# SeanNaren/deepspeech.pytorch

Measured on AMD Instinct MI355X. Metric: audio-seconds/sec (train step), higher is better.
Workload: dtype bf16

## Files before the change

deepspeech/pytorch_amd/_lib.py:

```python
import ctypes as C
import os

HERE = os.path.dirname(os.path.abspath(__file__))
LIB_PATH = os.path.join(HERE, "libds2hip.so")

F32, BF16 = 0, 1
CELL_GRU, CELL_LSTM, CELL_RNN_TANH = 0, 1, 2

_vp, _i, _l, _f, _ll = C.c_void_p, C.c_int, C.c_long, C.c_float, C.c_longlong

SIGNATURES = {
    "ds2_version": (_i, []),
    "ds2_error_string": (C.c_char_p, [_i]),
    "ds2_gemm_nt": (_i, [_i, _vp, _vp, _vp, _vp, _i, _i, _i, _l, _l, _l, _i, _i, _l, _l, _l, _l, _i, _vp]),
    "ds2_gemm_nt_coresident": (_i, [_i, _vp, _vp, _vp, _vp, _i, _i, _i, _l, _l, _l, _i, _i, _l, _l, _l, _l, _i, _vp]),
    "ds2_gemm_nt_rows2": (_i, [_i, _vp, _vp, _i, _vp, _vp, _i, _i, _i, _l, _l, _l, _i, _i, _i, _vp]),
    "ds2_gemm8_nt": (_i, [_vp, _vp, _vp, _vp, _i, _i, _i, _l, _l, _l, _i, _vp]),
    "ds2_gemm8_tn_grouped": (_i, [_i, _vp, _vp, _vp, _vp, _vp, _vp, _vp, _vp, _vp, _vp, _vp, _i, _vp]),
    "ds2_gemm8_nt_rows": (_i, [_vp, _vp, _vp, _vp, _i, _i, _i, _l, _l, _l, _i, _vp, _i, _vp]),
    "ds2_gemm8_tn_grouped_rows": (_i, [_i, _vp, _vp, _vp, _vp, _vp, _vp, _vp, _vp, _vp, _vp, _vp, _i, _vp, _i, _vp]),
    "ds2_gemm8_wgrad_dx_rows": (_i, [_i, _vp, _vp, _vp, _vp, _vp, _vp, _vp, _vp, _vp, _vp, _vp, _i, _vp, _vp, _vp, _i, _i, _i, _l, _l, _l, _vp, _i, _vp]),
    "ds2_zero_pad_rows": (_i, [_i, _vp, _l, _i, _vp, _i, _i, _vp]),
    "ds2_gemm8_wgrad_dx": (_i, [_i, _vp, _vp, _vp, _vp, _vp, _vp, _vp, _vp, _vp, _vp, _vp, _i, _vp, _vp, _vp, _i, _i, _i, _l, _l, _l, _vp]),
    "ds2_norm_partials": (_i, [_l]),
    "ds2_bn_fwd": (_i, [_i, _i, _i, _vp, _vp, _l, _i, _l, _l, _i, _i, _i, _vp, _vp, _vp, _vp, _vp, _vp, _f, _f, _vp, _vp,
                        _vp, _vp, _vp, _vp]),
    "ds2_bn_bwd": (_i, [_i, _i, _vp, _vp, _vp, _l, _i, _l, _l, _l, _i, _i, _i, _vp, _vp, _vp, _vp, _vp, _vp, _vp, _vp, _vp]),
    "ds2_colsum": (_i, [_i, _vp, _l, _i, _l, _vp, _f, _vp, _vp]),
    "ds2_conv_rows": (_i, [_i, _vp, _vp]),
    "ds2_conv1_fwd": (_i, [_i, _vp, _vp, _vp, _vp, _vp, _i, _i, _i, _i, _vp]),
    "ds2_conv1_wgrad_ws_floats": (_l, [_i, _i, _i]),
    "ds2_conv1_wgrad": (_i, [_i, _vp, _vp, _vp, _i, _i, _i, _i, _vp, _vp]),
    "ds2_conv2_fwd_ws_bytes": (_l, [_i, _i, _i, _i]),
    "ds2_conv2_fwd": (_i, [_i, _vp, _vp, _vp, _vp, _vp, _i, _i, _i, _vp, _vp]),
    "ds2_conv2_dgrad": (_i, [_i, _vp, _vp, _vp, _vp, _i, _i, _i, _vp]),
    "ds2_conv2_wgrad_ws_floats": (_l, [_i, _i]),
    "ds2_conv2_wgrad": (_i, [_i, _vp, _vp, _vp, _i, _i, _i, _vp, _vp]),
    "ds2_rnn_gates": (_i, [_i]),
    "ds2_rnn_saved_planes": (_i, [_i]),
    "ds2_rnn_state_bytes": (_l, [_i, _i, _i]),
    "ds2_rnn_fwd": (_i, [_i, _i, _i, _i, _i, _i, _vp, _vp, _vp, _vp, _vp, _vp, _vp, _l, _vp, _vp, _vp, _vp, _vp]),
    "ds2_rnn_bwd": (_i, [_i, _i, _i, _i, _i, _i, _vp, _vp, _vp, _vp, _l, _vp, _vp, _vp, _vp, _vp, _vp, _vp, _vp, _vp]),
    "ds2_rnn_persist_plan": (_i, [_i, _i, _i, _i, _i, _i, C.c_uint, C.POINTER(_l)]),
    "ds2_rnn_persist_supported": (_i, [_i, _i, _i, _i, _i, C.c_uint]),
    "ds2_rnn_persist_shape_covered": (_i, [_i, _i, _i, _i, _i]),
    "ds2_rnn_persist_kind": (_i, [_i, _i, _i, _i, _i, C.c_uint]),
    "ds2_rnn_persist_ws_bytes": (_l, [_i, _i, _i, _i, _i, C.c_uint]),
    "ds2_rnn_persist_fwd": (_i, [_i, _i, _i, _i, _i, _i, _vp, _vp, _vp, _vp, _vp, _vp, _vp, _l, _vp, _vp, _vp, _vp, _vp, _vp, _vp]),
    "ds2_rnn_persist_bwd": (_i, [_i, _i, _i, _i, _i, _i, _vp, _vp, _vp, _vp, _l, _vp, _vp, _vp, _vp, _i, _vp, _vp, _vp, _vp]),
    "ds2_add2": (_i, [_i, _vp, _vp, _vp, _l, _vp]),
    "ds2_sum_slices": (_i, [_vp, _vp, _l, _i, _vp]),
    "ds2_transpose": (_i, [_i, _vp, _vp, _l, _i, _l, _l, _vp]),
    "ds2_split3_bf16": (_i, [_vp, _l, _l, _i, _i, _i, _vp, _l, _vp]),
    "ds2_cast_transpose_bf16": (_i, [_vp, _l, _i, _i, _i, _i, _i, _vp, _l, _vp, _l, _vp]),
    "ds2_small_weight_layouts": (_i, [_i, _vp, _vp, _vp, _i, _i, _vp, _vp, _vp, _vp, _vp, _vp, _vp]),
    "ds2_scale_by": (_i, [_vp, _vp, _l, _vp]),
    "ds2_copy_words": (_i, [_vp, _vp, _l, _vp]),
    "ds2_lookahead_fwd": (_i, [_i, _vp, _vp, _vp, _vp, _i, _i, _i, _i, _vp]),
    "ds2_lookahead_ws_floats": (_l, [_i, _i, _i, _i]),
    "ds2_lookahead_bwd": (_i, [_i, _vp, _vp, _vp, _vp, _vp, _vp, _i, _i, _i, _i, _vp, _vp]),
    "ds2_rnn_bias_grads": (_i, [_i, _i, _i, _i, _vp, _vp, _vp, _vp]),
    "ds2_fc_supported": (_i, [_i, _i]),
    "ds2_fc_fwd": (_i, [_vp, _l, _vp, _l, _vp, _l, _l, _i, _i, _vp]),
    "ds2_fc_bwd_partials": (_l, [_l, _l]),
    "ds2_fc_bwd": (_i, [_vp, _l, _vp, _l, _vp, _l, _vp, _l, _vp, _vp, _l, _i, _i, _l, _vp]),
    "ds2_softmax_rows": (_i, [_vp, _vp, _l, _i, _l, _l, _vp]),
    "ds2_opt_max_tensors": (_i, []),
    "ds2_clip_ws_floats": (_l, [_i, _vp]),
    "ds2_clip_coef": (_i, [_i, _vp, _vp, _f, _vp, _vp, _vp]),
    "ds2_opt_multi": (_i, [_i, _i, _vp, _vp, _vp, _vp, _vp, _vp, _i, _vp, _vp]),
    "ds2_opt_matrix": (_i, [_i, _vp, _vp, _vp, _vp, _i, _i, _i, _i, _i, _vp, _l, _vp, _l, _vp, _i, _vp, _vp]),
    "ds2_opt_matrices": (_i, [_i, _i] + [_vp] * 13 + [_vp, _i, _vp, _vp]),
    "ds2_spect_frames": (_i, [_i]),
    "ds2_spect_ws_bytes": (_l, [_i, _i]),
    "ds2_spectrogram": (_i, [_vp, _l, _vp, _i, _i, _vp, _i, _i, _vp, _vp, _vp]),
    "ds2_spectrogram_aug": (_i, [_vp, _l, _vp, _i, _i, _vp, _i, _i, _vp, _vp, _vp, _i, _vp, _i, _vp, _i, _vp, _vp]),
    "ds2_spec_augment_coef": (_i, [_vp, _i, _i, _i, _vp, _vp, _i, _vp, _vp]),
    "ds2_spec_augment": (_i, [_vp, _vp, _i, _i, _i, _vp, _vp, _vp, _i, _vp, _i, _vp]),
    "ds2_wsola_segments": (_i, [_i, _f]),
    "ds2_wsola_out_len": (_l, [_i, _f]),
    "ds2_wsola": (_i, [_vp, _l, _vp, _vp, _i, _vp, _l, _vp, _vp, _i, _vp]),
    "ds2_wave_ws_bytes": (_l, [_i]),
    "ds2_wave_energy": (_i, [_vp, _l, _vp, _i, _vp, _vp, _vp, _l, _vp, _vp, _vp, _vp]),
    "ds2_wave_mix": (_i, [_vp, _l, _vp, _i, _vp, _vp, _vp, _l, _vp, _vp, _vp, _vp, _l, _vp]),
    "ds2_greedy_decode":(_i, [_vp, _l, _l, _i, _i, _i, _vp, _i, _vp, _vp, _vp, _vp]),
    "ds2_beam_ws_bytes": (_l, [_i, _i, _i]),
    "ds2_beam_decode": (_i, [_vp, _l, _l, _i, _i, _i, _vp, _i, _i, _i, _f, _vp, _vp, _vp, _vp, _vp, _vp]),
    "ds2_beam_decode_lm": (_i, [_vp, _l, _l, _i, _i, _i, _vp, _i, _i, _i, _f, _i, _vp, _l, _vp, _l, _i, _i, _f, _f, _i,
                                _vp, _vp, _vp, _vp, _vp, _vp, _vp]),
    "ds2_beam_grid_ws_bytes": (_l, [_i, _i, _i, _i]),
    "ds2_beam_decode_lm_grid": (_i, [_vp, _l, _l, _i, _i, _i, _vp, _i, _i, _i, _f, _i, _vp, _l, _vp, _l, _i, _i, _i, _i, _vp, _vp,
                                     _vp, _vp, _vp, _vp, _vp, _vp, _vp]),
    "ds2_greedy_stream_feed": (_i, [_vp, _l, _l, _i, _i, _i, _vp, _i, _vp, _vp, _vp, _vp, _vp]),
    "ds2_beam_stream_bytes": (_l, [_i, _i, _i, _i]),
    "ds2_beam_stream_ws_bytes": (_l, [_i, _i]),
    "ds2_beam_stream_state_stride": (_l, [_i, _i]),
    "ds2_beam_stream_reset": (_i, [_vp, _i, _i, _i, _i, _vp, _vp]),
    "ds2_beam_stream_feed": (_i, [_vp, _l, _l, _i, _i, _i, _vp, _i, _i, _i, _f, _vp, _i, _vp, _vp, _l, _i, _vp, _vp, _vp, _vp]),
    "ds2_beam_stream_feed_lm": (_i, [_vp, _l, _l, _i, _i, _i, _vp, _i, _i, _i, _f, _i, _vp, _l, _vp, _l, _i, _i, _f, _f, _i,
                                     _vp, _i, _vp, _vp, _l, _i, _vp, _vp, _vp, _vp, _vp]),
    "ds2_stream_plan": (_i, [_l, _i, _i, _i, _vp]),
    "ds2_stream_state_bytes": (_l, [_i, _i, _i, _i, _i]),
    "ds2_stream_conv1": (_i, [_i, _vp, _vp, _vp, _vp, _vp, _vp, _vp, _vp, _vp, _vp, _i, _i, _i, _i, _i, _vp]),
    "ds2_stream_conv2": (_i, [_i, _vp, _vp, _vp, _vp, _vp, _vp, _vp, _vp, _vp, _vp, _i, _i, _i, _i, _i, _i, _vp]),
    "ds2_stream_lookahead": (_i, [_i, _vp, _vp, _vp, _vp, _vp, _vp, _i, _i, _i, _i, _i, _i, _vp]),
    "ds2_stream_conv1_rows": (_i, [_i, _vp, _vp, _vp, _vp, _vp, _vp, _vp, _vp, _vp, _i, _i, _i, _i, _vp]),
    "ds2_stream_conv2_rows": (_i, [_i, _vp, _vp, _vp, _vp, _vp, _vp, _vp, _vp, _vp, _i, _i, _i, _i, _i, _i, _vp]),
    "ds2_stream_lookahead_rows": (_i, [_i, _vp, _vp, _vp, _vp, _vp, _vp, _i, _i, _i, _i, _i, _i, _vp]),
    "ds2_error_counts": (_i, [_vp, _l, _vp, _i, _vp, _vp, _i, _i, _vp, _vp, _vp, _vp, _vp]),
    "ds2_ctc_ws_floats": (_l, [_i, _i, _i, _i]),
    "ds2_ctc_loss_grad": (_i, [_vp, _l, _vp, _vp, _vp, _vp, _i, _i, _i, _i, _i, _f, _vp, _vp, _vp, _l, _vp, _i, _vp]),
    "ds2_ctc_align_ws_bytes": (_l, [_i, _i, _i]),
    "ds2_ctc_align": (_i, [_vp, _l, _l, _i, _i, _i, _i, _vp, _vp, _vp, _vp, _i, _i, _vp, _vp, _vp, _vp, _vp, _vp, _vp]),
}



class PersistOpts(C.Structure):
    _fields_ = [("variant", C.c_uint), ("spin_limit", C.c_uint), ("startup_ms", C.c_uint)]


_lib = None


class Ds2HipError(RuntimeError):
    pass


def load():
    global _lib
    if _lib is not None:
        return _lib
    if not os.path.exists(LIB_PATH):
        raise Ds2HipError(
            "libds2hip.so not found at %s -- build it with `python -m deepspeech.pytorch_amd.build` "
            "(hipcc --offload-arch=gfx950).  There is no fallback path." % LIB_PATH)
    lib = C.CDLL(LIB_PATH)
    for name, (res, args) in SIGNATURES.items():
        fn = getattr(lib, name)
        fn.restype = res
        fn.argtypes = args
    _lib = lib
    return lib


def error_string(code):
    return load().ds2_error_string(int(code)).decode()


def call(name, *args):
    rc = getattr(load(), name)(*args)
    if rc != 0:
        raise Ds2HipError("%s failed with code %d: %s" % (name, rc, error_string(rc)))


def query(name, *args):
    return getattr(load(), name)(*args)
```

deepspeech/pytorch_amd/csrc/ds2_conv.hip:

```cpp
#include "ds2_common.h"

namespace {

constexpr int F0 = 161, F1 = 81, F2 = 41, CH = 32;
constexpr int K1F = 41, K1T = 11, K2F = 21, K2T = 11;

constexpr int C1_FB = 4, C1_TB = 64;
constexpr int C1_PR = (C1_FB - 1) * 2 + K1F;
constexpr int C1_PC = (C1_TB - 1) * 2 + K1T;
constexpr int C1_PCP = C1_PC + 1;

__device__ __forceinline__ void conv1_load_patch(float* patch, const float* __restrict__ xn, int T, int f_base, int t_base,
                                                 int tid, int nthreads, int f0) {
  for (int i = tid; i < C1_PR * C1_PC; i += nthreads) {
    const int pr = i / C1_PC, pc = i - pr * C1_PC;
    const int fi = f_base + pr, ti = t_base + pc;
    const bool ok = fi >= 0 && fi < f0 && ti >= 0 && ti < T;
    const float v = xn[(long)min(max(fi, 0), f0 - 1) * T + min(max(ti, 0), T - 1)];
    patch[pr * C1_PCP + pc] = ok ? v : 0.f;
  }
}

template <typename T>
__global__ void __launch_bounds__(256) k_conv1_fwd(const float* __restrict__ x, const float* __restrict__ w1k,
// ... 652 lines not shown
    cur.j = q0 - cur.n * NJ;
  }
  cur = next_live(cur);
  int b = 0;
  if (cur.n < N) {
    const CwdNext first = plan(cur, 0);
    cwd_dma_dy<KSN, 0>(first); cwd_dma_dy<KSN, 1>(first); cwd_dma_dy<KSN, 2>(first);
    if constexpr (KSN > 3) cwd_dma_dy<KSN, 3>(first);
    if constexpr (KSN > 4) cwd_dma_dy<KSN, 4>(first);
    if constexpr (KSN > 5) cwd_dma_dy<KSN, 5>(first);
    if constexpr (KSN > 6) cwd_dma_dy<KSN, 6>(first);
    if constexpr (KSN > 7) cwd_dma_dy<KSN, 7>(first);
    cwd_dma_x<KSN, 0>(first); cwd_dma_x<KSN, 1>(first); cwd_dma_x<KSN, 2>(first);
  }
  while (cur.n < N) {
    Cursor nc = cur;
    advance(nc);
    nc = next_live(nc);
    const CwdNext nx = plan(nc, b ^ 1);
    CWD_WAIT_VM0();
    __builtin_amdgcn_sched_barrier(0);
    __builtin_amdgcn_s_barrier();
    __builtin_amdgcn_sched_barrier(0);
    const uint32_t aA = la + b * BUF, aB = lb + b * BUF;
#define CWD_FIRST(IDX) CWD_READ(fa[0], fb[0], 0, IDX);
    CWD_FIRST(0) CWD_FIRST(1) CWD_FIRST(2) CWD_FIRST(3) CWD_FIRST(4) CWD_FIRST(5) CWD_FIRST(6)
    CWD_FIRST(7) CWD_FIRST(8) CWD_FIRST(9) CWD_FIRST(10) CWD_FIRST(11) CWD_FIRST(12) CWD_FIRST(13)
#undef CWD_FIRST
    cwd_kstep<KSN, 0>(acc, fa, fb, aA, aB, nx);
    cwd_kstep<KSN, 1>(acc, fa, fb, aA, aB, nx);
    cwd_kstep<KSN, 2>(acc, fa, fb, aA, aB, nx);
    if constexpr (KSN > 3) cwd_kstep<KSN, 3>(acc, fa, fb, aA, aB, nx);
    if constexpr (KSN > 4) cwd_kstep<KSN, 4>(acc, fa, fb, aA, aB, nx);
    if constexpr (KSN > 5) cwd_kstep<KSN, 5>(acc, fa, fb, aA, aB, nx);
    if constexpr (KSN > 6) cwd_kstep<KSN, 6>(acc, fa, fb, aA, aB, nx);
    if constexpr (KSN > 7) cwd_kstep<KSN, 7>(acc, fa, fb, aA, aB, nx);
    cur = nc;
    b ^= 1;
  }
#pragma unroll
  for (int r = 0; r < R; ++r)
#pragma unroll
    for (int i = 0; i < 3; ++i) {
      const int kt = wave + 4 * i;
      if (kt < K2T && kf0 + 2 * r < K2F) {
        float* out = partial + (((long)split * K2F + (kf0 + 2 * r)) * K2T + kt) * (CH * CH);
#pragma unroll
        for (int e = 0; e < 16; ++e) out[mma32_row(e, lane) * 32 + li] = acc[r][i][e];
      }
    }
}

struct RTapArgs {
  const bf16_t* X;
  const bf16_t* W;
  const float* bias;
  const int* lens;
  const float* Pin;
  float* Pout;
  bf16_t* Y;
  int N, Tp, Fin, Fout;
  int KF, WSF, WQ;
  int ISF, IQ, PF;
  int U, OSF, OQ;
};
constexpr int RT_FB = 4, RT_TB = 32, RT_PC = RT_TB + K2T - 1;
constexpr int RT_KFM = 11, RT_PR = RT_FB - 1 + RT_KFM;
constexpr int RT_PCD = 48, RT_ROWB = RT_PCD * CH * 2;
constexpr int RT_PATCH = RT_PR * RT_ROWB;
constexpr int RT_RED = 4 * RT_FB * 4096;
constexpr int RT_SMEM = 2 * RT_PATCH + RT_RED;
#define RT_RD128(dst, addr, off) asm volatile("ds_read_b128 %0, %1 offset:%2" : "=v"(dst) : "v"(addr), "i"(off))

struct RtNext {
  __amdgpu_buffer_rsrc_t rx;
  unsigned char* patch;
  int n, ub, tb;
  int Fin, Tp, PF, ISF, IQ;
  int wave, lane;
};
template <int PR, int I>
__device__ __forceinline__ void rt_dma_piece(const RtNext& nx) {
  constexpr int k = I % 3;
  const int pr = nx.wave + 4 * (I / 3);
  if (pr < PR) {
    const int fi = (nx.ub * RT_FB + pr - nx.PF) * nx.ISF + nx.IQ;
    const bool row_ok = nx.n >= 0 && fi >= 0 && fi < nx.Fin;
    const int soff = __builtin_amdgcn_readfirstlane(row_ok ? (nx.n * nx.Fin + fi) * (nx.Tp * CH * 2) : 0);
    const int pc = 16 * k + (nx.lane >> 2), ti = nx.tb * RT_TB - 5 + pc;
    const int voff = (row_ok && pc < RT_PC && (unsigned)ti < (unsigned)nx.Tp) ? ti * (CH * 2) + (((nx.lane & 3) ^ (nx.lane >> 4)) << 4) : CW_OOB;
    __builtin_amdgcn_raw_ptr_buffer_load_lds(nx.rx, (cw_lds_ptr_t)(nx.patch + pr * RT_ROWB + k * 1024), 16, voff, soff, 0, 0);
  }
}
template <int PR, int I>
__device__ __forceinline__ void rt_dma_all(const RtNext& nx) {
  rt_dma_piece<PR, I>(nx);
  if constexpr (I + 1 < 12) rt_dma_all<PR, I + 1>(nx);
}
constexpr int RT_AH = 4;
template <int ST>
__device__ __forceinline__ void rt_prefetch(uint4 (&bq)[RT_AH + 1], const uint32_t (&aj)[6]) {
  RT_RD128(bq[ST], aj[ST % 6], (ST / 6) * RT_ROWB);
  if constexpr (ST + 1 < RT_AH) rt_prefetch<ST + 1>(bq, aj);
}
template <int KF, int ST>
__device__ __forceinline__ void rt_step(ds2_f32x16 (&acc)[RT_FB], const uint4 (&A)[KF][6], uint4 (&bq)[RT_AH + 1], const uint32_t (&aj)[6],
                                        const RtNext& nx) {
  constexpr int PR = RT_FB - 1 + KF, NS = PR * 6, rho = ST / 6, j = ST % 6;
  if constexpr (ST + RT_AH < NS) RT_RD128(bq[(ST + RT_AH) % (RT_AH + 1)], aj[(ST + RT_AH) % 6], ((ST + RT_AH) / 6) * RT_ROWB);
  constexpr int left = RT_AH < NS - 1 - ST ? RT_AH : NS - 1 - ST;
  if constexpr (left >= 4) asm volatile("s_waitcnt lgkmcnt(4)" ::: "memory");
  else if constexpr (left == 3) asm volatile("s_waitcnt lgkmcnt(3)" ::: "memory");
  else if constexpr (left == 2) asm volatile("s_waitcnt lgkmcnt(2)" ::: "memory");
  else if constexpr (left == 1) asm volatile("s_waitcnt lgkmcnt(1)" ::: "memory");
  else asm volatile("s_waitcnt lgkmcnt(0)" ::: "memory");
  __builtin_amdgcn_sched_barrier(0);
#pragma unroll
  for (int fl = 0; fl < RT_FB; ++fl) {
    const int m = rho - fl;
    if (m >= 0 && m < KF) Mma<bf16_t>::mma32(acc[fl], A[m][j], bq[ST % (RT_AH + 1)]);
  }
  if constexpr (ST % 6 == 3 && ST >= 9 && (ST - 9) / 6 < 12) rt_dma_piece<PR, (ST - 9) / 6>(nx);
  __builtin_amdgcn_sched_barrier(0);
  if constexpr (ST + 1 < NS) rt_step<KF, ST + 1>(acc, A, bq, aj, nx);
}

template <int KF>
__global__ void __launch_bounds__(256, 1) k_conv_rtap(RTapArgs a) {
  extern __shared__ __attribute__((aligned(16))) unsigned char rsm[];
  float* red = reinterpret_cast<float*>(rsm + 2 * RT_PATCH);
  const int tid = threadIdx.x, lane = tid & 63, wave = __builtin_amdgcn_readfirstlane(tid >> 6);
  const int li = lane & 31, lq = lane >> 5;
  const int i0 = wave < 2 ? 6 * wave : 12 + 5 * (wave - 2), icnt = wave < 2 ? 6 : 5;
  uint4 A[KF][6];
  const uint32_t lds0 = (uint32_t)(uintptr_t)(__attribute__((address_space(3))) unsigned char*)rsm;
  uint32_t boff[6];
#pragma unroll
  for (int j = 0; j < 6; ++j) {
    const int item = i0 + min(j, icnt - 1), kt = item >> 1, half = item & 1;
    const int p = li + kt;
    boff[j] = lds0 + p * (CH * 2) + (((half * 2 + lq) ^ ((p >> 2) & 3)) << 4);
#pragma unroll
    for (int m = 0; m < KF; ++m) {
      const uint4 wv = *reinterpret_cast<const uint4*>(a.W + (((long)(m * a.WSF + a.WQ) * K2T + kt) * CH + li) * CH + half * 16 + lq * 8);
      A[m][j] = j < icnt ? wv : make_uint4(0u, 0u, 0u, 0u);
    }
  }
#ifndef DS2_RTAP_VKEEP
#define DS2_RTAP_VKEEP 24
#endif
#pragma unroll
  for (int m = 0; m < KF; ++m)
#pragma unroll
    for (int j = 0; j < 6; ++j)
      if (m * 6 + j >= DS2_RTAP_VKEEP) {
        typedef __attribute__((ext_vector_type(4))) unsigned int u4v;
        u4v v = __builtin_bit_cast(u4v, A[m][j]);
        asm volatile("" : "+a"(v));
        A[m][j] = __builtin_bit_cast(uint4, v);
      }
  constexpr int PR = RT_FB - 1 + KF;
  constexpr int NPIECE = 12;
  const int nub = ds2_cdiv_dev(a.U, RT_FB), ntb = ds2_cdiv_dev(a.Tp, RT_TB);
  const int total = a.N * nub * ntb;
  RtNext nx;
  nx.rx = __builtin_amdgcn_make_buffer_rsrc((void*)a.X, 0, a.N * a.Fin * a.Tp * CH * 2, 0x00020000);
  nx.Fin = a.Fin; nx.Tp = a.Tp; nx.PF = a.PF; nx.ISF = a.ISF; nx.IQ = a.IQ;
  nx.wave = wave; nx.lane = lane;
  auto aim = [&](int tile, int buf) {
    const bool any = tile < total;
    const int tt = any ? tile : 0;
    nx.tb = tt % ntb;
    nx.ub = (tt / ntb) % nub;
    nx.n = any ? tt / (ntb * nub) : -1;
    nx.patch = rsm + buf * RT_PATCH;
  };

  int tile = blockIdx.x;
  if (tile < total) {
    aim(tile, 0);
    rt_dma_all<PR, 0>(nx);
  }
  __syncthreads();
  int buf = 0;
  for (; tile < total; tile += gridDim.x, buf ^= 1) {
    const int tb = tile % ntb, ub = (tile / ntb) % nub, n = tile / (ntb * nub);
    const int next = tile + gridDim.x;
    aim(next, buf ^ 1);
    float4 pin[4];
    {
      const int u = ub * RT_FB + wave, t = tb * RT_TB + li;
      const bool have = a.Pin != nullptr && u < a.U && t < a.Tp;
      const float* src = a.Pin + (((long)n * a.U + min(u, a.U - 1)) * a.Tp + min(t, a.Tp - 1)) * CH + 4 * lq;
#pragma unroll
      for (int g = 0; g < 4; ++g) pin[g] = have ? *reinterpret_cast<const float4*>(src + 8 * g) : make_float4(0.f, 0.f, 0.f, 0.f);
    }
    ds2_f32x16 acc[RT_FB];
#pragma unroll
    for (int fl = 0; fl < RT_FB; ++fl)
#pragma unroll
      for (int r = 0; r < 16; ++r) acc[fl][r] = 0.f;
    {
      uint4 bq[RT_AH + 1];
      uint32_t aj[6];
#pragma unroll
      for (int j = 0; j < 6; ++j) aj[j] = boff[j] + buf * RT_PATCH;
      __builtin_amdgcn_sched_barrier(0);
      rt_prefetch<0>(bq, aj);
      rt_step<KF, 0>(acc, A, bq, aj, nx);
    }
#pragma unroll
    for (int fl = 0; fl < RT_FB; ++fl)
#pragma unroll
      for (int g = 0; g < 4; ++g)
        *reinterpret_cast<float4*>(red + (((wave * RT_FB + fl) * 4 + g) * 64 + lane) * 4) =
            make_float4(acc[fl][4 * g], acc[fl][4 * g + 1], acc[fl][4 * g + 2], acc[fl][4 * g + 3]);
    asm volatile("s_waitcnt vmcnt(0)" ::: "memory");
    __syncthreads();
    {
      const int u = ub * RT_FB + wave, t = tb * RT_TB + li;
      float o[16];
#pragma unroll
      for (int g = 0; g < 4; ++g) {
        float4 s4 = *reinterpret_cast<const float4*>(red + (((0 * RT_FB + wave) * 4 + g) * 64 + lane) * 4);
#pragma unroll
        for (int w = 1; w < 4; ++w) {
          const float4 q4 = *reinterpret_cast<const float4*>(red + (((w * RT_FB + wave) * 4 + g) * 64 + lane) * 4);
          s4.x += q4.x; s4.y += q4.y; s4.z += q4.z; s4.w += q4.w;
        }
        o[4 * g] = s4.x; o[4 * g + 1] = s4.y; o[4 * g + 2] = s4.z; o[4 * g + 3] = s4.w;
      }
      if (u < a.U && t < a.Tp) {
        const long pidx = (((long)n * a.U + u) * a.Tp + t) * CH + 4 * lq;
        if (a.Pin) {
#pragma unroll
          for (int g = 0; g < 4; ++g) {
            o[4 * g] += pin[g].x; o[4 * g + 1] += pin[g].y; o[4 * g + 2] += pin[g].z; o[4 * g + 3] += pin[g].w;
          }
        }
        if (a.Pout) {
#pragma unroll
          for (int g = 0; g < 4; ++g)
            *reinterpret_cast<float4*>(a.Pout + pidx + 8 * g) = make_float4(o[4 * g], o[4 * g + 1], o[4 * g + 2], o[4 * g + 3]);
        } else {
          const bool live = a.lens ? (t < a.lens[n]) : true;
          bf16_t* dst = a.Y + (((long)n * a.Fout + u * a.OSF + a.OQ) * a.Tp + t) * CH + 4 * lq;
#pragma unroll
          for (int g = 0; g < 4; ++g) {
            float e[4];
#pragma unroll
            for (int c = 0; c < 4; ++c) e[c] = live ? o[4 * g + c] + (a.bias ? a.bias[8 * g + 4 * lq + c] : 0.f) : 0.f;
            *reinterpret_cast<uint2*>(dst + 8 * g) = make_uint2(cvt_pk_bf16(e[0], e[1]), cvt_pk_bf16(e[2], e[3]));
          }
        }
      }
    }
    asm volatile("s_waitcnt lgkmcnt(0)" ::: "memory");
    __builtin_amdgcn_sched_barrier(0);
    __builtin_amdgcn_s_barrier();
    __builtin_amdgcn_sched_barrier(0);
  }
}

template <int KF>
int conv_rtap_launch_kf(const RTapArgs& a, hipStream_t st) {
  static bool attr[DS2_MAX_DEVICES];
  if (ds2_first_use_on_device(attr)) (void)hipFuncSetAttribute((const void*)k_conv_rtap<KF>, hipFuncAttributeMaxDynamicSharedMemorySize, RT_SMEM);
  const long total = (long)a.N * ds2_cdiv(a.U, RT_FB) * ds2_cdiv(a.Tp, RT_TB);
  const int cus = ds2_cu_count();
  hipLaunchKernelGGL(k_conv_rtap<KF>, dim3((unsigned)(total < cus ? total : cus)), dim3(256), RT_SMEM, st, a);
  DS2_CHECK_LAUNCH();
  return 0;
}
int conv_rtap_launch(const RTapArgs& a, hipStream_t st) {
  if (a.KF == 11) return conv_rtap_launch_kf<11>(a, st);
  if (a.KF == 10) return conv_rtap_launch_kf<10>(a, st);
  return DS2_ERR_ARG;
}

template <typename T, int NT>
int conv_tap_launch_nt(const ConvTapArgs& a, hipStream_t st) {
  const int PR = (CT_UB - 1) * a.SF + a.KF, PC = CT_TB * NT + K2T - 1;
  const int shm = PR * PC * CT_POSB + 2 * CT_WST_BYTES;
  static int attr[DS2_MAX_DEVICES];
  int dev = 0;
  (void)hipGetDevice(&dev);
  dev = dev >= 0 && dev < DS2_MAX_DEVICES ? dev : 0;
  if (attr[dev] < shm) {
    (void)hipFuncSetAttribute((const void*)k_conv_tap<T, NT>, hipFuncAttributeMaxDynamicSharedMemorySize, shm);
    attr[dev] = shm;
  }
  dim3 grid(ds2_cdiv(a.Tp, CT_TB * NT), ds2_cdiv(a.U, CT_UB), a.N);
  hipLaunchKernelGGL((k_conv_tap<T, NT>), grid, dim3(256), shm, st, a);
  DS2_CHECK_LAUNCH();
  return 0;
}
template <typename T>
int conv_tap_launch(const ConvTapArgs& a, hipStream_t st) {
  const int PR = (CT_UB - 1) * a.SF + a.KF;
  if (PR * (2 * CT_TB + K2T - 1) * CT_POSB + 2 * CT_WST_BYTES <= 150 * 1024) return conv_tap_launch_nt<T, 2>(a, st);
  return conv_tap_launch_nt<T, 1>(a, st);
}

}

static bool conv_geometry(int f0, int& f1, int& f2) {
  f1 = (f0 + 2 * 20 - K1F) / 2 + 1;
  f2 = (f1 + 2 * 10 - K2F) / 2 + 1;
  return f0 >= 1 && f1 >= 1 && f2 >= 1;
}

extern "C" {

int ds2_conv_rows(int F0, int* F1_out, int* F2_out) {
  int f1, f2;
  DS2_REQUIRE(conv_geometry(F0, f1, f2), DS2_ERR_ARG);
  if (F1_out) *F1_out = f1;
  if (F2_out) *F2_out = f2;
  return 0;
}

int ds2_conv1_fwd(int dtype, const float* x, const float* w1k, const float* b1, const int* lens, void* y1, int N, int F0_, int T,
                  int Tp, ds2_stream_t st_) {
  hipStream_t st = (hipStream_t)st_;
  DS2_REQUIRE(dtype == DS2_F32 || dtype == DS2_BF16, DS2_ERR_DTYPE);
  int f1, f2;
  DS2_REQUIRE(N > 0 && T > 0 && Tp == (T + 2 * 5 - 10 - 1) / 2 + 1 && conv_geometry(F0_, f1, f2), DS2_ERR_ARG);
  dim3 grid(ds2_cdiv(Tp, C1_TB), ds2_cdiv(f1, C1_FB), N);
  if (dtype == DS2_F32) {
    hipLaunchKernelGGL(k_conv1_fwd<float>, grid, dim3(256), 0, st, x, w1k, b1, lens, (float*)y1, N, T, Tp, F0_, f1);
  } else if (F0_ != F0) {
    hipLaunchKernelGGL(k_conv1_fwd<bf16_t>, grid, dim3(256), 0, st, x, w1k, b1, lens, (bf16_t*)y1, N, T, Tp, F0_, f1);
  } else {
    const int ntb = ds2_cdiv(Tp, M1_TB);
    const long total = (long)N * ntb * 9;
    const int cus = ds2_cu_count();
    hipLaunchKernelGGL(k_conv1_fwd_mfma, dim3((unsigned)(total < cus ? total : cus)), dim3(256), 0, st, x, w1k, b1, lens, (bf16_t*)y1, N,
                       T, Tp, ntb);
  }
  DS2_CHECK_LAUNCH();
  return 0;
}

static int conv1_wgrad_blocks(int N, int f1, int Tp) {
  long total = (long)N * ds2_cdiv(f1, C1_FB) * ds2_cdiv(Tp, C1_TB);
  return (int)(total < C1W_MAXBLOCKS ? total : C1W_MAXBLOCKS);
}
static int conv1_wgrad_mfma_blocks(int N, int Tp) {
  const long total = (long)N * ds2_cdiv(Tp, M1_TB) * 9;
  const int cus = ds2_cu_count();
  return (int)(total < cus ? total : cus);
}
long ds2_conv1_wgrad_ws_floats(int N, int F0_, int Tp) {
  int f1, f2;
  if (!conv_geometry(F0_, f1, f2)) return 0;
  const long P = conv1_wgrad_blocks(N, f1, Tp);
  return P * (K1F * K1T * CH) + (long)ds2_norm_partials(P) * (K1F * K1T * CH);
}
int ds2_conv1_wgrad(int dtype, const float* x, const void* dy1, float* dw1k, int N, int F0_, int T, int Tp, float* ws,
                    ds2_stream_t st_) {
  hipStream_t st = (hipStream_t)st_;
  DS2_REQUIRE(dtype == DS2_F32 || dtype == DS2_BF16, DS2_ERR_DTYPE);
  int f1, f2;
  DS2_REQUIRE(conv_geometry(F0_, f1, f2), DS2_ERR_ARG);
  int P = conv1_wgrad_blocks(N, f1, Tp);
  const int ncf = ds2_cdiv(f1, C1_FB), nct = ds2_cdiv(Tp, C1_TB);
  if (dtype == DS2_F32) {
    hipLaunchKernelGGL(k_conv1_wgrad<float>, dim3(P), dim3(C1W_THREADS), 0, st, x, (const float*)dy1, ws, N, T, Tp, nct, ncf, F0_, f1);
  } else if (F0_ != F0) {
    hipLaunchKernelGGL(k_conv1_wgrad<bf16_t>, dim3(P), dim3(C1W_THREADS), 0, st, x, (const bf16_t*)dy1, ws, N, T, Tp, nct, ncf, F0_, f1);
  } else {
    static bool attr[DS2_MAX_DEVICES];
    if (ds2_first_use_on_device(attr))
      (void)hipFuncSetAttribute((const void*)k_conv1_wgrad_mfma, hipFuncAttributeMaxDynamicSharedMemorySize, M1W_SMEM);
    P = conv1_wgrad_mfma_blocks(N, Tp) < P ? conv1_wgrad_mfma_blocks(N, Tp) : P;
    hipLaunchKernelGGL(k_conv1_wgrad_mfma, dim3(P), dim3(256), M1W_SMEM, st, x, (const bf16_t*)dy1, ws, N, T, Tp, ds2_cdiv(Tp, M1_TB));
  }
  DS2_CHECK_LAUNCH();
  const int C = K1F * K1T * CH;
  return ds2_colsum(DS2_F32, ws, P, C, C, dw1k, 1.0f, ws + (long)P * C, st_);
}

long ds2_conv2_fwd_ws_bytes(int dtype, int N, int F0_, int Tp) { return (dtype == DS2_BF16 && F0_ == F0) ? (long)N * F2 * Tp * CH * 4 : 0; }
int ds2_conv2_fwd(int dtype, const void* a1, const void* w2t, const float* b2, const int* lens, void* y2, int N, int F0_, int Tp, void* ws,
                  ds2_stream_t st_) {
  hipStream_t st = (hipStream_t)st_;
  DS2_REQUIRE(dtype == DS2_F32 || dtype == DS2_BF16, DS2_ERR_DTYPE);
  int f1, f2;
  DS2_REQUIRE(N > 0 && Tp > 0 && conv_geometry(F0_, f1, f2), DS2_ERR_ARG);
  if (dtype == DS2_F32 || F0_ != F0 || (long)N * F1 * Tp * CH * 2 >= (long)CW_OOB) {
    ConvTapArgs a{a1, w2t, b2, lens, y2, N, Tp, f1, f2, K2F, 2, 10, f2, 1, 0};
    return dtype == DS2_F32 ? conv_tap_launch<float>(a, st) : conv_tap_launch<bf16_t>(a, st);
  }
  DS2_REQUIRE(ws != nullptr, DS2_ERR_ARG);
  RTapArgs e{(const bf16_t*)a1, (const bf16_t*)w2t, nullptr, nullptr, nullptr, (float*)ws, nullptr, N, Tp, F1, F2, 11, 2, 0, 2, 0, 5, F2, 1, 0};
  RTapArgs o{(const bf16_t*)a1, (const bf16_t*)w2t, b2, lens, (const float*)ws, nullptr, (bf16_t*)y2, N, Tp, F1, F2, 10, 2, 1, 2, 1, 5, F2, 1, 0};
  const int rc = conv_rtap_launch(e, st);
  return rc ? rc : conv_rtap_launch(o, st);
}

int ds2_conv2_dgrad(int dtype, const void* dy2, const void* w2d_even, const void* w2d_odd, void* da1, int N, int F0_, int Tp,
                    ds2_stream_t st_) {
  hipStream_t st = (hipStream_t)st_;
  DS2_REQUIRE(dtype == DS2_F32 || dtype == DS2_BF16, DS2_ERR_DTYPE);
  int f1, f2;
  DS2_REQUIRE(N > 0 && Tp > 0 && conv_geometry(F0_, f1, f2), DS2_ERR_ARG);
  if (dtype == DS2_BF16 && F0_ == F0 && (long)N * F1 * Tp * CH * 2 < (long)CW_OOB) {
    RTapArgs e{(const bf16_t*)dy2, (const bf16_t*)w2d_even, nullptr, nullptr, nullptr, nullptr, (bf16_t*)da1, N, Tp, F2, F1, 11, 1, 0, 1, 0, 5, 41, 2, 0};
    RTapArgs o{(const bf16_t*)dy2, (const bf16_t*)w2d_odd, nullptr, nullptr, nullptr, nullptr, (bf16_t*)da1, N, Tp, F2, F1, 10, 1, 0, 1, 0, 4, 40, 2, 1};
    const int rc = conv_rtap_launch(e, st);
    return rc ? rc : conv_rtap_launch(o, st);
  }
  ConvTapArgs e{dy2, w2d_even, nullptr, nullptr, da1, N, Tp, f2, f1, 11, 1, 5, (f1 + 1) / 2, 2, 0};
  ConvTapArgs o{dy2, w2d_odd, nullptr, nullptr, da1, N, Tp, f2, f1, 10, 1, 4, f1 / 2, 2, 1};
  if (dtype == DS2_F32) {
    const int rc = conv_tap_launch<float>(e, st);
    return (rc || f1 / 2 == 0) ? rc : conv_tap_launch<float>(o, st);
  }
  const int rc = conv_tap_launch<bf16_t>(e, st);
  return (rc || f1 / 2 == 0) ? rc : conv_tap_launch<bf16_t>(o, st);
}

long ds2_conv2_wgrad_ws_floats(int N, int Tp) {
  (void)N; (void)Tp;
  const long C = (long)K2F * K2T * CH * CH;
  static_assert(CWR_SPLITS >= CW_SPLITS, "sized for the larger split count of the two kernels");
  return (long)CWR_SPLITS * C + (long)ds2_norm_partials(CWR_SPLITS) * C;
}
int ds2_conv2_wgrad(int dtype, const void* dy2, const void* a1, float* dw2t, int N, int F0_, int Tp, float* ws, ds2_stream_t st_) {
  hipStream_t st = (hipStream_t)st_;
  DS2_REQUIRE(dtype == DS2_F32 || dtype == DS2_BF16, DS2_ERR_DTYPE);
  int f1, f2;
  DS2_REQUIRE(conv_geometry(F0_, f1, f2), DS2_ERR_ARG);
  dim3 grid(K2F, CW_SPLITS);
  const bool general = dtype == DS2_F32 || F0_ != F0 || (long)N * F1 * Tp * CH * 2 >= (long)CW_OOB;
  if (dtype == DS2_F32) {
    hipLaunchKernelGGL(k_conv2_wgrad<float>, grid, dim3(256), 0, st, (const float*)dy2, (const float*)a1, ws, N, Tp, f1, f2);
  } else if (general) {
    hipLaunchKernelGGL(k_conv2_wgrad<bf16_t>, grid, dim3(256), 0, st, (const bf16_t*)dy2, (const bf16_t*)a1, ws, N, Tp, f1, f2);
  } else {
    static bool attr[DS2_MAX_DEVICES];
    constexpr int smem = cwd_smem_bytes(CWD_KSN);
    if (ds2_first_use_on_device(attr))
      (void)hipFuncSetAttribute((const void*)k_conv2_wgrad_bf16d<CWD_KSN>, hipFuncAttributeMaxDynamicSharedMemorySize, smem);
    hipLaunchKernelGGL(k_conv2_wgrad_bf16d<CWD_KSN>, dim3(8 * CWD_UNITS_PER_XCD), dim3(256), smem, st, (const bf16_t*)dy2, (const bf16_t*)a1, ws, N,
                       Tp, CWR_SPLITS);
  }
  DS2_CHECK_LAUNCH();
  const int C = K2F * K2T * CH * CH;
  const int splits = general ? CW_SPLITS : CWR_SPLITS;
  return ds2_colsum(DS2_F32, ws, splits, C, C, dw2t, 1.0f, ws + (long)splits * C, st_);
}

}
```

deepspeech/pytorch_amd/csrc/ds2_norm.hip:

```cpp
#include "ds2_common.h"

namespace {

constexpr int NORM_RY = 8;
constexpr int NORM_CX = 32;

struct RowMap {
  int F, Tp;
  __device__ __forceinline__ void nt(long row, int& n, int& t) const {
    t = (int)(row % Tp);
    n = (int)(row / ((long)F * Tp));
  }
};

__device__ __forceinline__ float bn_affine(float x, float sc, float sh) { return __builtin_fmaf(x, sc, sh); }
__device__ __forceinline__ bool hardtanh_open(float y) { return y > 0.f && y < 20.f; }
__device__ __forceinline__ float bn_dx(float g, float xh, float sc, float k1, float k2) { return sc * __builtin_fmaf(-xh, k2, g - k1); }

struct RedMap {
  int cpb, rpx, chunk, rsub;
  bool ok;
  __device__ __forceinline__ RedMap(int chunks) {
    cpb = chunks < NORM_CX ? chunks : NORM_CX;
    rpx = NORM_CX / cpb;
    const int tx = threadIdx.x;
    rsub = tx / cpb;
    chunk = blockIdx.x * cpb + tx % cpb;
    ok = rsub < rpx && chunk < chunks;
  }
  __device__ __forceinline__ long first_row() const { return ((long)blockIdx.y * NORM_RY + threadIdx.y) * rpx + rsub; }
  __device__ __forceinline__ long row_step() const { return (long)gridDim.y * NORM_RY * rpx; }
};
template <int V>
__device__ __forceinline__ void red_block(float (*red)[NORM_CX * V + 1], const RedMap& m, const float (&v)[V], float (&out)[V]) {
  __syncthreads();
#pragma unroll
  for (int i = 0; i < V; ++i) red[threadIdx.y][threadIdx.x * V + i] = v[i];
  __syncthreads();
  if (threadIdx.y == 0 && m.rsub == 0) {
#pragma unroll
    for (int i = 0; i < V; ++i) {
      float a = 0.f;
      for (int k = 0; k < m.rpx; ++k)
#pragma unroll
        for (int y = 0; y < NORM_RY; ++y) a += red[y][(threadIdx.x + k * m.cpb) * V + i];
      out[i] = a;
    }
  }
}

template <typename T, bool SQ>
__global__ void __launch_bounds__(NORM_RY* NORM_CX) k_colstats(const T* __restrict__ X, long R, int C, long ld,
                                                                float* __restrict__ psum, float* __restrict__ psq) {
  constexpr int V = Vec16<T>::N;
  __shared__ float red[NORM_RY][NORM_CX * V + 1];
  const RedMap m(C / V);
  float s[V], q[V];
#pragma unroll
  for (int i = 0; i < V; ++i) s[i] = q[i] = 0.f;
  if (m.ok) {
    for (long r = m.first_row(); r < R; r += m.row_step()) {
      float v[V];
      Vec16<T>::load(X + r * ld + (long)m.chunk * V, v);
#pragma unroll
      for (int i = 0; i < V; ++i) {
        s[i] += v[i];
        if (SQ) q[i] += v[i] * v[i];
      }
    }
  }
  float o[V];
  red_block<V>(red, m, s, o);
  if (threadIdx.y == 0 && m.rsub == 0 && m.ok) {
#pragma unroll
    for (int i = 0; i < V; ++i) psum[(long)blockIdx.y * C + (long)m.chunk * V + i] = o[i];
  }
  if (SQ) {
    red_block<V>(red, m, q, o);
    if (threadIdx.y == 0 && m.rsub == 0 && m.ok) {
#pragma unroll
      for (int i = 0; i < V; ++i) psq[(long)blockIdx.y * C + (long)m.chunk * V + i] = o[i];
    }
  }
}

constexpr int FIN_COLS = 32, FIN_SLICES = 8;
template <int NA>
__device__ __forceinline__ void finalize_sums(const float* const (&arr)[NA], int P, int C, int c, int py, double (&tot)[NA]) {
  __shared__ double sh[NA][FIN_SLICES][FIN_COLS];
  double acc[NA];
#pragma unroll
  for (int a = 0; a < NA; ++a) acc[a] = 0.0;
  if (c < C) {
#pragma unroll 8
    for (int p = py; p < P; p += FIN_SLICES) {
#pragma unroll
      for (int a = 0; a < NA; ++a) acc[a] += (double)arr[a][(long)p * C + c];
    }
  }
#pragma unroll
  for (int a = 0; a < NA; ++a) sh[a][py][threadIdx.x & (FIN_COLS - 1)] = acc[a];
  __syncthreads();
#pragma unroll
  for (int a = 0; a < NA; ++a) {
    double t = 0.0;
    if (py == 0) {
#pragma unroll
      for (int q = 0; q < FIN_SLICES; ++q) t += sh[a][q][threadIdx.x & (FIN_COLS - 1)];
    }
    tot[a] = t;
  }
}

__global__ void __launch_bounds__(256) k_colsum_finalize(const float* __restrict__ psum, int P, int C, float* __restrict__ out,
                                                          float scale) {
  const int c = blockIdx.x * FIN_COLS + (threadIdx.x & (FIN_COLS - 1)), py = threadIdx.x / FIN_COLS;
  const float* const arr[1] = {psum};
  double tot[1];
  finalize_sums<1>(arr, P, C, c, py, tot);
  if (py == 0 && c < C) out[c] = (float)(tot[0] * (double)scale);
}

__global__ void k_bn_finalize(const float* __restrict__ psum, const float* __restrict__ psq, int P, int C, double count,
                              const float* __restrict__ gamma, const float* __restrict__ beta, float eps,
                              float momentum, float* __restrict__ running_mean, float* __restrict__ running_var,
                              long long* __restrict__ num_batches_tracked, float* __restrict__ mean_out,
                              float* __restrict__ rstd_out, float* __restrict__ scale_out, float* __restrict__ shift_out) {
  const int c = blockIdx.x * FIN_COLS + (threadIdx.x & (FIN_COLS - 1)), py = threadIdx.x / FIN_COLS;
  if (blockIdx.x == 0 && threadIdx.x == 0 && num_batches_tracked) *num_batches_tracked += 1;
  const float* const arr[2] = {psum, psq};
  double tot[2];
  finalize_sums<2>(arr, P, C, c, py, tot);
  if (py != 0 || c >= C) return;
  const double s = tot[0], q = tot[1];
  double mean = s / count;
  double var = q / count - mean * mean;
  if (var < 0.0) var = 0.0;
  double rstd = 1.0 / sqrt(var + (double)eps);
  mean_out[c] = (float)mean;
  rstd_out[c] = (float)rstd;
  float sc = (float)((double)gamma[c] * rstd);
  scale_out[c] = sc;
  shift_out[c] = (float)((double)beta[c] - mean * (double)gamma[c] * rstd);
  if (running_mean) {
    double unb = count > 1.0 ? var * (count / (count - 1.0)) : var;
    running_mean[c] = (float)((1.0 - (double)momentum) * (double)running_mean[c] + (double)momentum * mean);
    running_var[c] = (float)((1.0 - (double)momentum) * (double)running_var[c] + (double)momentum * unb);
  }
}

__global__ void k_bn_eval_coeffs(int C, const float* __restrict__ gamma, const float* __restrict__ beta,
                                 const float* __restrict__ running_mean, const float* __restrict__ running_var, float eps,
                                 float* __restrict__ scale_out, float* __restrict__ shift_out) {
  int c = blockIdx.x * blockDim.x + threadIdx.x;
  if (c >= C) return;
  double rstd = 1.0 / sqrt((double)running_var[c] + (double)eps);
  scale_out[c] = (float)((double)gamma[c] * rstd);
  shift_out[c] = (float)((double)beta[c] - (double)running_mean[c] * (double)gamma[c] * rstd);
}

template <typename T, bool CONV, bool SEQ_OUT, bool CENTRED = false>
__global__ void __launch_bounds__(256) k_bn_apply(const T* __restrict__ X, T* __restrict__ Y, long R, int C, long ldx,
                                                   long ldy, const float* __restrict__ scale,
                                                   const float* __restrict__ shift, const float* __restrict__ mean,
                                                   const float* __restrict__ beta, RowMap rm,
                                                   const int* __restrict__ lens, int N) {
  constexpr int V = Vec16<T>::N;
  const int chunks = C / V;
  const long total = R * chunks;
  for (long e = (long)blockIdx.x * blockDim.x + threadIdx.x; e < total; e += (long)gridDim.x * blockDim.x) {
    long r = e / chunks;
    int c0 = (int)(e % chunks) * V;
    float v[V];
    bool live = true;
    int n = 0, t = 0;
    if (CONV) {
      rm.nt(r, n, t);
      live = t < lens[n];
    }
    if (live) {
      Vec16<T>::load(X + r * ldx + c0, v);
#pragma unroll
      for (int i = 0; i < V; ++i) {
        float y = CENTRED ? __builtin_fmaf(v[i] - mean[c0 + i], scale[c0 + i], beta[c0 + i]) : bn_affine(v[i], scale[c0 + i], shift[c0 + i]);
        if (CONV) y = fminf(fmaxf(y, 0.f), 20.f);
        v[i] = y;
      }
    } else {
#pragma unroll
      for (int i = 0; i < V; ++i) v[i] = 0.f;
    }
    if (SEQ_OUT) {
      int f = (int)((r / rm.Tp) % rm.F);
      Vec16<T>::store(Y + ((long)t * N + n) * ldy + (long)f * C + c0, v);
    } else {
      Vec16<T>::store(Y + r * ldy + c0, v);
    }
  }
}

template <typename T, bool CONV, bool SEQ_IN>
__device__ __forceinline__ bool load_gated(const T* __restrict__ G, const T* __restrict__ X, long r, int c0, int C,
                                           long ldg, long ldx, const float* __restrict__ scale,
                                           const float* __restrict__ shift, const float* __restrict__ mean,
                                           const float* __restrict__ rstd, const RowMap& rm, const int* __restrict__ lens,
                                           int N, float (&g)[Vec16<T>::N], float (&xh)[Vec16<T>::N]) {
  constexpr int V = Vec16<T>::N;
  int n = 0, t = 0, f = 0;
  if (CONV) {
    const unsigned ur = (unsigned)r, q = ur / (unsigned)rm.Tp;
    t = (int)(ur - q * (unsigned)rm.Tp);
    n = (int)(q / (unsigned)rm.F);
    f = (int)(q - (unsigned)n * (unsigned)rm.F);
  }
  const int len = CONV ? lens[n] : 0;
  float x[V];
  Vec16<T>::load(X + r * ldx + c0, x);
  if (SEQ_IN) {
    Vec16<T>::load(G + ((long)t * N + n) * ldg + (long)f * C + c0, g);
  } else {
    Vec16<T>::load(G + r * ldg + c0, g);
  }
  if (CONV && t >= len) return false;
#pragma unroll
  for (int i = 0; i < V; ++i) {
    if (CONV) {
      if (!hardtanh_open(bn_affine(x[i], scale[c0 + i], shift[c0 + i]))) g[i] = 0.f;
    }
    xh[i] = (x[i] - mean[c0 + i]) * rstd[c0 + i];
  }
  return true;
}

template <typename T, bool CONV, bool SEQ_IN>
__global__ void __launch_bounds__(NORM_RY* NORM_CX)
    k_bn_bwd_reduce(const T* __restrict__ G, const T* __restrict__ X, long R, int C, long ldg, long ldx,
                    const float* __restrict__ scale, const float* __restrict__ shift, const float* __restrict__ mean,
                    const float* __restrict__ rstd, RowMap rm, const int* __restrict__ lens, int N,
                    float* __restrict__ psum_g, float* __restrict__ psum_gx) {
  constexpr int V = Vec16<T>::N;
  __shared__ float red[NORM_RY][NORM_CX * V + 1];
  const RedMap m(C / V);
  float s[V], q[V];
#pragma unroll
  for (int i = 0; i < V; ++i) s[i] = q[i] = 0.f;
  if (m.ok) {
    for (long r = m.first_row(); r < R; r += m.row_step()) {
      float g[V], xh[V];
      if (load_gated<T, CONV, SEQ_IN>(G, X, r, m.chunk * V, C, ldg, ldx, scale, shift, mean, rstd, rm, lens, N, g, xh)) {
#pragma unroll
        for (int i = 0; i < V; ++i) {
          s[i] += g[i];
          q[i] += g[i] * xh[i];
        }
      }
    }
  }
  float o[V];
  red_block<V>(red, m, s, o);
  if (threadIdx.y == 0 && m.rsub == 0 && m.ok) {
#pragma unroll
    for (int i = 0; i < V; ++i) psum_g[(long)blockIdx.y * C + (long)m.chunk * V + i] = o[i];
  }
  red_block<V>(red, m, q, o);
  if (threadIdx.y == 0 && m.rsub == 0 && m.ok) {
#pragma unroll
    for (int i = 0; i < V; ++i) psum_gx[(long)blockIdx.y * C + (long)m.chunk * V + i] = o[i];
  }
}

__global__ void k_bn_bwd_finalize(const float* __restrict__ psum_g, const float* __restrict__ psum_gx, int P, int C,
                                  double count, float* __restrict__ dgamma, float* __restrict__ dbeta,
                                  float* __restrict__ c1, float* __restrict__ c2) {
  const int c = blockIdx.x * FIN_COLS + (threadIdx.x & (FIN_COLS - 1)), py = threadIdx.x / FIN_COLS;
  const float* const arr[2] = {psum_g, psum_gx};
  double tot[2];
  finalize_sums<2>(arr, P, C, c, py, tot);
  if (py != 0 || c >= C) return;
  const double s = tot[0], q = tot[1];
  dbeta[c] = (float)s;
  dgamma[c] = (float)q;
  c1[c] = (float)(s / count);
  c2[c] = (float)(q / count);
}

template <typename T, bool CONV, bool SEQ_IN>
__global__ void __launch_bounds__(NORM_RY* NORM_CX)
    k_bn_bwd_apply_cols(const T* __restrict__ G, const T* __restrict__ X, T* __restrict__ DX, long R, int C, long ldg, long ldx,
                        long lddx, const float* __restrict__ scale, const float* __restrict__ shift,
                        const float* __restrict__ mean, const float* __restrict__ rstd, const float* __restrict__ c1,
                        const float* __restrict__ c2, RowMap rm, const int* __restrict__ lens, int N) {
  constexpr int V = Vec16<T>::N;
  const RedMap m(C / V);
  if (!m.ok) return;
  const int c0 = m.chunk * V;
  float sc[V], sh[V], mu[V], rs[V], k1[V], k2[V];
#pragma unroll
  for (int i = 0; i < V; ++i) {
    sc[i] = scale[c0 + i];
    sh[i] = CONV ? shift[c0 + i] : 0.f;
    mu[i] = mean[c0 + i];
    rs[i] = rstd[c0 + i];
    k1[i] = c1[c0 + i];
    k2[i] = c2[c0 + i];
  }
  const long step = m.row_step();
  auto addr = [&](long r, int& t, int& len, const T*& gp) {
    int n = 0, f = 0;
    t = 0;
    if (CONV) {
      const unsigned ur = (unsigned)r, q = ur / (unsigned)rm.Tp;
      t = (int)(ur - q * (unsigned)rm.Tp);
      n = (int)(q / (unsigned)rm.F);
      f = (int)(q - (unsigned)n * (unsigned)rm.F);
    }
    len = CONV ? lens[n] : 0;
    gp = SEQ_IN ? G + ((long)t * N + n) * ldg + (long)f * C + c0 : G + r * ldg + c0;
  };
  auto finish = [&](long r, int t, int len, float (&x)[V], float (&g)[V]) {
    float o[V];
    if (CONV && t >= len) {
#pragma unroll
      for (int i = 0; i < V; ++i) o[i] = 0.f;
    } else {
#pragma unroll
      for (int i = 0; i < V; ++i) {
        float gi = g[i];
        if (CONV) {
          if (!hardtanh_open(bn_affine(x[i], sc[i], sh[i]))) gi = 0.f;
        }
        const float xh = (x[i] - mu[i]) * rs[i];
        o[i] = bn_dx(gi, xh, sc[i], k1[i], k2[i]);
      }
    }
    Vec16<T>::store(DX + r * lddx + c0, o);
  };
  long r = m.first_row();
  for (; r + step < R; r += 2 * step) {
    int t0, t1, l0, l1;
    const T *g0p, *g1p;
    addr(r, t0, l0, g0p);
    addr(r + step, t1, l1, g1p);
    float x0[V], x1[V], g0[V], g1[V];
    Vec16<T>::load(X + r * ldx + c0, x0);
    Vec16<T>::load(X + (r + step) * ldx + c0, x1);
    Vec16<T>::load(g0p, g0);
    Vec16<T>::load(g1p, g1);
    finish(r, t0, l0, x0, g0);
    finish(r + step, t1, l1, x1, g1);
  }
  if (r < R) {
    int t0, l0;
    const T* g0p;
    addr(r, t0, l0, g0p);
    float x0[V], g0[V];
    Vec16<T>::load(X + r * ldx + c0, x0);
    Vec16<T>::load(g0p, g0);
    finish(r, t0, l0, x0, g0);
  }
}

inline int norm_grid_y(long R, int col_blocks = 1) {
  long gy = (R + NORM_RY - 1) / NORM_RY;
  long cap = 1024 / (col_blocks < 1 ? 1 : col_blocks);
  if (cap < 256) cap = 256;
  if (gy > cap) gy = cap;
  if (gy < 1) gy = 1;
  return (int)gy;
}

template <typename T>
int colstats_impl(const void* X, long R, int C, long ld, float* psum, float* psq, int* P_out, hipStream_t st) {
  constexpr int V = Vec16<T>::N;
  DS2_REQUIRE(C % V == 0 && ld % V == 0, DS2_ERR_ALIGN);
  dim3 blk(NORM_CX, NORM_RY);
  dim3 grd(ds2_cdiv(C / V, NORM_CX), norm_grid_y(R, ds2_cdiv(C / V, NORM_CX)));
  if (psq)
    hipLaunchKernelGGL((k_colstats<T, true>), grd, blk, 0, st, (const T*)X, R, C, ld, psum, psq);
  else
    hipLaunchKernelGGL((k_colstats<T, false>), grd, blk, 0, st, (const T*)X, R, C, ld, psum, psq);
  *P_out = grd.y;
  DS2_CHECK_LAUNCH();
  return 0;
}

inline int apply_grid(long total) {
  long g = (total + 255) / 256;
  if (g > 256 * 8) g = 256 * 8;
  if (g < 1) g = 1;
  return (int)g;
}

}

extern "C" {

int ds2_norm_partials(long R) { return norm_grid_y(R); }

int ds2_colsum(int dtype, const void* X, long R, int C, long ld, float* out, float scale, float* ws, ds2_stream_t st_) {
  hipStream_t st = (hipStream_t)st_;
  int P = 0, rc;
  if (dtype == DS2_F32)
    rc = colstats_impl<float>(X, R, C, ld, ws, nullptr, &P, st);
  else
    rc = colstats_impl<bf16_t>(X, R, C, ld, ws, nullptr, &P, st);
  if (rc) return rc;
  hipLaunchKernelGGL(k_colsum_finalize, dim3(ds2_cdiv(C, FIN_COLS)), dim3(256), 0, st, ws, P, C, out, scale);
  DS2_CHECK_LAUNCH();
  return 0;
}

int ds2_bn_fwd(int dtype, int mode, int training, const void* X, void* Y, long R, int C, long ldx, long ldy, int F, int Tp,
               int N, const int* lens, const float* gamma, const float* beta, float* running_mean, float* running_var,
               long long* num_batches_tracked, float eps, float momentum, float* save_mean, float* save_rstd,
               float* save_scale, float* save_shift, float* ws, ds2_stream_t st_) {
  hipStream_t st = (hipStream_t)st_;
  DS2_REQUIRE(dtype == DS2_F32 || dtype == DS2_BF16, DS2_ERR_DTYPE);
  DS2_REQUIRE(mode >= 0 && mode <= 2, DS2_ERR_ARG);
  DS2_REQUIRE(mode == 0 || R < (1L << 31), DS2_ERR_ARG);
  int rc, P = 0;
  if (training) {
    float* psum = ws;
    float* psq = ws + (long)norm_grid_y(R) * C;
    rc = dtype == DS2_F32 ? colstats_impl<float>(X, R, C, ldx, psum, psq, &P, st)
                          : colstats_impl<bf16_t>(X, R, C, ldx, psum, psq, &P, st);
    if (rc) return rc;
    hipLaunchKernelGGL(k_bn_finalize, dim3(ds2_cdiv(C, FIN_COLS)), dim3(256), 0, st, psum, psq, P, C, (double)R, gamma, beta,
                       eps, momentum, running_mean, running_var, num_batches_tracked, save_mean, save_rstd, save_scale,
                       save_shift);
  } else {
    hipLaunchKernelGGL(k_bn_eval_coeffs, dim3(ds2_cdiv(C, 128)), dim3(128), 0, st, C, gamma, beta, running_mean,
                       running_var, eps, save_scale, save_shift);
  }
  DS2_CHECK_LAUNCH();
  RowMap rm{F, Tp};
  const int V = dtype == DS2_F32 ? 4 : 8;
  DS2_REQUIRE(C % V == 0 && ldx % V == 0 && ldy % V == 0, DS2_ERR_ALIGN);
  dim3 g(apply_grid(R * (C / V))), b(256);
#define LAUNCH_APPLY(TT)                                                                                              \
  if (mode == 0 && training && R == 1)                                                                                \
    hipLaunchKernelGGL((k_bn_apply<TT, false, false, true>), g, b, 0, st, (const TT*)X, (TT*)Y, R, C, ldx, ldy,        \
                       save_scale, save_shift, save_mean, beta, rm, lens, N);                                         \
  else if (mode == 0)                                                                                                 \
    hipLaunchKernelGGL((k_bn_apply<TT, false, false>), g, b, 0, st, (const TT*)X, (TT*)Y, R, C, ldx, ldy, save_scale,  \
                       save_shift, save_mean, beta, rm, lens, N);                                                     \
  else if (mode == 1)                                                                                                 \
    hipLaunchKernelGGL((k_bn_apply<TT, true, false>), g, b, 0, st, (const TT*)X, (TT*)Y, R, C, ldx, ldy, save_scale,   \
                       save_shift, save_mean, beta, rm, lens, N);                                                     \
  else                                                                                                                \
    hipLaunchKernelGGL((k_bn_apply<TT, true, true>), g, b, 0, st, (const TT*)X, (TT*)Y, R, C, ldx, ldy, save_scale,    \
                       save_shift, save_mean, beta, rm, lens, N);
  if (dtype == DS2_F32) {
    LAUNCH_APPLY(float)
  } else {
    LAUNCH_APPLY(bf16_t)
  }
#undef LAUNCH_APPLY
  DS2_CHECK_LAUNCH();
  return 0;
}

int ds2_bn_bwd(int dtype, int mode, const void* G, const void* X, void* DX, long R, int C, long ldg, long ldx, long lddx,
               int F, int Tp, int N, const int* lens, const float* save_mean, const float* save_rstd,
               const float* save_scale, const float* save_shift, float* dgamma, float* dbeta, float* ws, ds2_stream_t st_) {
  hipStream_t st = (hipStream_t)st_;
  DS2_REQUIRE(dtype == DS2_F32 || dtype == DS2_BF16, DS2_ERR_DTYPE);
  DS2_REQUIRE(mode >= 0 && mode <= 2, DS2_ERR_ARG);
  DS2_REQUIRE(mode == 0 || R < (1L << 31), DS2_ERR_ARG);
  const int V = dtype == DS2_F32 ? 4 : 8;
  DS2_REQUIRE(C % V == 0 && ldx % V == 0 && ldg % V == 0 && lddx % V == 0, DS2_ERR_ALIGN);
  RowMap rm{F, Tp};
  const int P = norm_grid_y(R, ds2_cdiv(C / V, NORM_CX));
  float* ps = ws;
  float* pq = ws + (long)P * C;
  float* c1 = pq + (long)P * C;
  float* c2 = c1 + C;
  dim3 blk(NORM_CX, NORM_RY), grd(ds2_cdiv(C / V, NORM_CX), P);
#define LAUNCH_RED(TT, CV, SI)                                                                                          \
  hipLaunchKernelGGL((k_bn_bwd_reduce<TT, CV, SI>), grd, blk, 0, st, (const TT*)G, (const TT*)X, R, C, ldg, ldx,          \
                     save_scale, save_shift, save_mean, save_rstd, rm, lens, N, ps, pq)
  const int acb = ds2_cdiv(C / V, NORM_CX), arpx = NORM_CX / (C / V < NORM_CX ? C / V : NORM_CX);
  long agy = ds2_cdiv(R, (long)NORM_RY * arpx * 2);
  if (agy > 2048 / acb) agy = 2048 / acb;
  if (agy < 1) agy = 1;
  const dim3 agrd(acb, (unsigned)agy);
#define LAUNCH_APP(TT, CV, SI)                                                                                          \
  hipLaunchKernelGGL((k_bn_bwd_apply_cols<TT, CV, SI>), agrd, blk, 0, st, (const TT*)G, (const TT*)X, (TT*)DX, R, C, ldg, \
                     ldx, lddx, save_scale, save_shift, save_mean, save_rstd, c1, c2, rm, lens, N)
#define BOTH(WHICH)                                        \
  if (dtype == DS2_F32) {                                  \
    if (mode == 0) WHICH(float, false, false);             \
    else if (mode == 1) WHICH(float, true, false);         \
    else WHICH(float, true, true);                         \
  } else {                                                 \
    if (mode == 0) WHICH(bf16_t, false, false);            \
    else if (mode == 1) WHICH(bf16_t, true, false);        \
    else WHICH(bf16_t, true, true);                        \
  }
  BOTH(LAUNCH_RED)
  DS2_CHECK_LAUNCH();
  hipLaunchKernelGGL(k_bn_bwd_finalize, dim3(ds2_cdiv(C, FIN_COLS)), dim3(256), 0, st, ps, pq, P, C, (double)R, dgamma, dbeta,
                     c1, c2);
  DS2_CHECK_LAUNCH();
  BOTH(LAUNCH_APP)
  DS2_CHECK_LAUNCH();
#undef BOTH
#undef LAUNCH_RED
#undef LAUNCH_APP
  return 0;
}

}
```

deepspeech/pytorch_amd/model.py:

```python
import math
from typing import List

import numpy as np
import torch
import torch.nn as nn

from . import ops
from ._lib import Ds2HipError

try:
    import pytorch_lightning as pl
    _Base = pl.LightningModule
except Exception:
    pl = None

    class _Base(nn.Module):

        def save_hyperparameters(self, *a, **k):
            import inspect
            frame = inspect.currentframe().f_back
            try:
                names = [n for n in inspect.signature(type(self).__init__).parameters if n != "self"]
                self._hparams = {n: frame.f_locals[n] for n in names if n in frame.f_locals}
            finally:
                del frame

        @property
        def hparams(self):
            return getattr(self, "_hparams", {})

        def log(self, *a, **k):
            pass

        @property
        def device(self):
            return next(self.parameters()).device

        @classmethod
        def load_from_checkpoint(cls, checkpoint_path, map_location=None, strict=True, **overrides):
            ckpt = torch.load(checkpoint_path, map_location=map_location or "cpu", weights_only=False)
            hp = dict(ckpt.get("hyper_parameters", {}))
            hp.update(overrides)
            model = cls(**hp)
            model.load_state_dict(ckpt["state_dict"], strict=strict)
            return model

try:
    from omegaconf import OmegaConf

    def _cfg_type_name(cfg):
        t = OmegaConf.get_type(cfg)
        return getattr(t, "__name__", str(t))
except Exception:
    def _cfg_type_name(cfg):
        return type(cfg).__name__

from .configs import AdamConfig, BiDirectionalConfig, SGDConfig, SpectConfig, UniDirectionalConfig, rnn_kind

import os

WGRAD_WITH_DX = os.environ.get("DS2_WGRAD_WITH_DX", "1") not in ("", "0")

COMPOSITE_NODE = {"": None, "0": False}.get(os.environ.get("DS2_COMPOSITE_NODE", ""), True)
PER_LAYER_NODES_FOR_DDP = [False]


PAD_HIDDEN = os.environ.get("DS2_PAD_HIDDEN", "1") != "0"


def _padded_hidden(H, kind, precision, bidirectional=None):
    base = (int(H) + 15) // 16 * 16
    if not PAD_HIDDEN or base < 200 or kind not in ("gru", "lstm", "rnn"):
        return base
    try:
        from ._lib import query
        dt_ = ops.dt(torch.bfloat16 if str(precision) in ("16", "bf16", "16-mixed", "bf16-mixed") else torch.float32)
        cell = ops.CELLS[kind]
        dirs = (2, 1) if bidirectional is None else ((2,) if bidirectional else (1,))
        for w in range(base, int(base * 1.5) + 1, 16):
            if any(query("ds2_rnn_persist_shape_covered", dt_, cell, D_, 1, w) for D_ in dirs):
                return w
    except Exception:
        pass
    return base


def _data_parallel_active():
    if PER_LAYER_NODES_FOR_DDP[0]:
        return True
    try:
        import torch.distributed as _dist
        return _dist.is_available() and _dist.is_initialized() and _dist.get_world_size() > 1
    except Exception:
        return False


FP32_WGRAD_TN = os.environ.get("DS2_FP32_WGRAD_TN", "1") != "0"

ROW_LISTS = os.environ.get("DS2_ROW_LISTS", "1") != "0"
ROW_LIST_MIN_PADDING = 0.97

N_FREQ_CONV2 = 41
RNN_INPUT = 32 * N_FREQ_CONV2
RNN_INPUT_LD = 1344


def _round64(n):
    return (n + 63) // 64 * 64


class SequenceWise(nn.Module):
    def __init__(self, module):
        super().__init__()
        self.module = module


class MaskConv(nn.Module):
    def __init__(self, seq_module):
        super().__init__()
        self.seq_module = seq_module


class _RNNParams(nn.Module):

    def __init__(self, kind, input_size, hidden_size, bidirectional):
        super().__init__()
        g = ops.GATES[kind]
        for suf in [""] + (["_reverse"] if bidirectional else []):
            self.register_parameter("weight_ih_l0" + suf, nn.Parameter(torch.empty(g * hidden_size, input_size)))
            self.register_parameter("weight_hh_l0" + suf, nn.Parameter(torch.empty(g * hidden_size, hidden_size)))
            self.register_parameter("bias_ih_l0" + suf, nn.Parameter(torch.empty(g * hidden_size)))
            self.register_parameter("bias_hh_l0" + suf, nn.Parameter(torch.empty(g * hidden_size)))
        stdv = 1.0 / math.sqrt(hidden_size) if hidden_size > 0 else 0
        for w in self.parameters():
            nn.init.uniform_(w, -stdv, stdv)


class BatchRNN(nn.Module):
    def __init__(self, input_size, hidden_size, kind, bidirectional=False, batch_norm=True):
        super().__init__()
        self.input_size, self.hidden_size, self.bidirectional, self.kind = input_size, hidden_size, bidirectional, kind
        self.batch_norm = SequenceWise(nn.BatchNorm1d(input_size)) if batch_norm else None
        self.rnn = _RNNParams(kind, input_size, hidden_size, bidirectional)
        self.num_directions = 2 if bidirectional else 1


class Lookahead(nn.Module):
    def __init__(self, n_features, context):
        super().__init__()
        assert context > 0
        self.context, self.n_features = context, n_features
        self.conv = nn.Conv1d(n_features, n_features, kernel_size=context, stride=1, groups=n_features, padding=0, bias=False)


class _WeightCache:

    def __init__(self):
        self._store = {}
        self.epoch = 0

    def get(self, key, params, builder):
        ver = (self.epoch,) + tuple((p._version, p.data_ptr()) for p in params)
        hit = self._store.get(key)
        if hit is not None and hit[0] == ver:
            return hit[1]
        with torch.no_grad():
            val = builder()
        self._store[key] = (ver, val)
        return val

    def _ver(self, params):
        return (self.epoch,) + tuple((p._version, p.data_ptr()) for p in params)

    def valid(self, key, params):
        hit = self._store.get(key)
        return hit is not None and hit[0] == self._ver(params)

    def put(self, key, params, val, epoch=None):
        ver = self._ver(params)
        if epoch is not None:
            ver = (epoch,) + ver[1:]
        self._store[key] = (ver, val)

    def clear(self):
        self._store.clear()


def _wgrad_splitk(M, N, K):
    tiles = ((M + 127) // 128) * ((N + 127) // 128)
    if tiles >= 128:
        return 1
    return max(1, min(8, 768 // max(tiles, 1), K // (64 * 32)))


def _pad_gate_rows(w, G, H, Hp):
    if Hp == H:
        return w
    out = w.new_zeros((G, Hp) + tuple(w.shape[1:]))
    out[:, :H] = w.reshape((G, H) + tuple(w.shape[1:]))
    return out.reshape((G * Hp,) + tuple(w.shape[1:]))


def _pad_cols(w, Cp):
    if w.shape[-1] == Cp:
        return w
    out = w.new_zeros(tuple(w.shape[:-1]) + (Cp,))
    out[..., :w.shape[-1]] = w
    return out


def _unpad_gate_rows(g, G, H, Hp):
    if Hp == H:
        return g
    return g.reshape((G, Hp) + tuple(g.shape[1:]))[:, :H].reshape((G * H,) + tuple(g.shape[1:])).contiguous()


def _bn_seq_fwd(bn, w, b, X, Xh, R, Ct, Cp, training):
    if Ct == Cp:
        return ops.bn_fwd(X, 0, training, w.detach(), b.detach(), bn.running_mean, bn.running_var, bn.num_batches_tracked, R, Ct,
                          X.stride(0), Xh, Xh.stride(0), eps=bn.eps, momentum=bn.momentum)
    g, be = w.new_ones(Cp), w.new_zeros(Cp)
    rm, rv = w.new_zeros(Cp), w.new_ones(Cp)
    g[:Ct], be[:Ct], rm[:Ct], rv[:Ct] = w.detach(), b.detach(), bn.running_mean, bn.running_var
    sv = ops.bn_fwd(X, 0, training, g, be, rm, rv, bn.num_batches_tracked, R, Cp, X.stride(0), Xh, Xh.stride(0), eps=bn.eps,
                    momentum=bn.momentum)
    if training:
        bn.running_mean.copy_(rm[:Ct])
        bn.running_var.copy_(rv[:Ct])
    return sv


def _bn_seq_bwd(G, X, DX, sv, R, Ct, Cp):
    dg, db = ops.bn_bwd(G, X, DX, 0, sv, R, Cp, G.stride(0), X.stride(0), DX.stride(0))
    return (dg, db) if Ct == Cp else (dg[:Ct].contiguous(), db[:Ct].contiguous())


def _perm_cols_to_internal(w):
    g, rin = w.shape
    out = w.new_zeros((g, _round64(rin)))
    out[:, :rin] = w.reshape(g, 32, rin // 32).permute(0, 2, 1).reshape(g, rin)
    return out


def _perm_cols_to_reference(w, rin=RNN_INPUT):
    g = w.shape[0]
    return w[:, :rin].reshape(g, rin // 32, 32).permute(0, 2, 1).reshape(g, rin)


class _ConvStackFn(torch.autograd.Function):

    @staticmethod
    def forward(ctx, x, w1, b1, g1, be1, w2, b2, g2, be2, mod, lens_dev, Tp, dtype, training):
        N, T = x.shape[0], x.shape[3]
        c = mod._cache
        bn1, bn2 = mod.conv.seq_module[1], mod.conv.seq_module[4]
        w1k = c.get("w1k", [w1], lambda: w1.detach().reshape(32, 451).t().contiguous())
        w2t = c.get(("w2t", dtype), [w2], lambda: w2.detach().permute(2, 3, 0, 1).contiguous().to(dtype))
        x = x.contiguous().float()
        F0, F1, F2, rin, rld = mod._F0, mod._F1, mod._F2, mod._rnn_in, mod._rnn_ld
        if x.shape[2] != F0:
            raise ValueError("this model was built for %d frequency bins (SpectConfig: sample_rate * window_size / 2 + 1), got input "
                             "with %d" % (F0, x.shape[2]))
        y1 = ops.conv1_fwd(x, w1k, b1.detach(), lens_dev, Tp, dtype)
        R1 = N * F1 * Tp
        a1 = torch.empty_like(y1)
        sv1 = ops.bn_fwd(y1, 1, training, g1.detach(), be1.detach(), bn1.running_mean, bn1.running_var,
                         bn1.num_batches_tracked, R1, 32, 32, a1, 32, F=F1, Tp=Tp, N=N, lens=lens_dev, eps=bn1.eps,
                         momentum=bn1.momentum)
        y2 = ops.conv2_fwd(a1, w2t, b2.detach(), lens_dev, F0)
        R2 = N * F2 * Tp
        x0 = torch.empty((Tp * N, rld), dtype=dtype, device=x.device)
        if rld > rin:
            x0[:, rin:].zero_()
        sv2 = ops.bn_fwd(y2, 2, training, g2.detach(), be2.detach(), bn2.running_mean, bn2.running_var,
                         bn2.num_batches_tracked, R2, 32, 32, x0, rld, F=F2, Tp=Tp, N=N, lens=lens_dev, eps=bn2.eps,
                         momentum=bn2.momentum)
        ctx.mod, ctx.dims, ctx.sv = mod, (N, T, Tp, dtype), (sv1, sv2)
        ctx.save_for_backward(x, y1, a1, y2, lens_dev, w2)
        return x0

    @staticmethod
    def backward(ctx, dx0):
        x, y1, a1, y2, lens_dev, w2 = ctx.saved_tensors
        N, T, Tp, dtype = ctx.dims
        sv1, sv2 = ctx.sv
        c = ctx.mod._cache
        dx0 = dx0.contiguous().to(dtype)
        F0, F1, F2, rld = ctx.mod._F0, ctx.mod._F1, ctx.mod._F2, ctx.mod._rnn_ld
        R1, R2 = N * F1 * Tp, N * F2 * Tp
        dy2 = torch.empty_like(y2)
        dg2, dbe2 = ops.bn_bwd(dx0, y2, dy2, 2, sv2, R2, 32, rld, 32, 32, F=F2, Tp=Tp, N=N, lens=lens_dev)
        w2d = c.get(("w2d", dtype), [w2], lambda: [
            w2.detach()[:, :, q::2, :].flip(2, 3).permute(2, 3, 1, 0).contiguous().to(dtype) for q in (0, 1)])
        da1 = ops.conv2_dgrad(dy2, w2d[0], w2d[1], F0)
        dy1 = torch.empty_like(y1)
        dg1, dbe1 = ops.bn_bwd(da1, y1, dy1, 1, sv1, R1, 32, 32, 32, 32, F=F1, Tp=Tp, N=N, lens=lens_dev)
        db1 = ops.colsum(dy1.view(R1, 32))
        dw1k = ops.conv1_wgrad(x, dy1, Tp)
        dw1 = dw1k.t().reshape(32, 1, 41, 11).contiguous()
        db2 = ops.colsum(dy2.view(R2, 32))
        dw2 = ops.conv2_wgrad(dy2, a1, F0).view(21, 11, 32, 32).permute(2, 3, 0, 1).contiguous()
        return (None, dw1, db1, dg1, dbe1, dw2, db2, dg2, dbe2, None, None, None, None, None)


def _layer_param_count(layer):
    return (2 if layer.batch_norm is not None else 0) + 4 * layer.num_directions


_ROWS_STAGING, _CTC_STAGING = ops.PinnedRing(), ops.PinnedRing()


def _frame_rows(output_lengths, Tp, N, dev):
    ol = output_lengths.numpy().astype(np.int32)
    n_valid = int(np.minimum(ol, Tp).sum())
    if not ROW_LISTS or n_valid >= ROW_LIST_MIN_PADDING * Tp * N or n_valid == 0:
        return output_lengths.to(dev, torch.int32, non_blocking=True), None
    rows = np.flatnonzero(np.arange(Tp, dtype=np.int32)[:, None] < ol[None, :]).astype(np.int32)
    both = _ROWS_STAGING.stage(dev, [ol, rows])
    return both[:N], both[N:]


def _rnn_layer_forward(mod, li, X, lens_dev, N, Tp, dtype, training, h0, c0, lparams, rows=None):
    c = mod._cache
    R = Tp * N
    layer = mod.rnns[li]
    kind, Ht, D = layer.kind, layer.hidden_size, layer.num_directions
    H = mod._Hp
    G = ops.GATES[kind]
    first = li == 0
    I = mod._rnn_ld if first else H
    has_bn = layer.batch_norm is not None
    bn_w, bn_b = (lparams[0], lparams[1]) if has_bn else (None, None)
    wts = lparams[2 if has_bn else 0:]
    wih = [wts[4 * d + 0] for d in range(D)]
    whh = [wts[4 * d + 1] for d in range(D)]
    bih = [wts[4 * d + 2] for d in range(D)]
    bhh = [wts[4 * d + 3] for d in range(D)]

    def build_ih():
        w = torch.cat([_pad_gate_rows(p.detach(), G, Ht, H) for p in wih], 0)
        w = _perm_cols_to_internal(w) if first else _pad_cols(w, H)
        out = ops.empty_padded(w.shape[0], w.shape[1], dtype, w.device)
        out.copy_(w)
        return out
    Wih = c.get(("wih", li, dtype), wih, build_ih)
    Whh = c.get(("whh", li, dtype), whh, lambda: torch.stack(
        [_pad_gate_rows(_pad_cols(p.detach(), H), G, Ht, H) for p in whh], 0).to(dtype).contiguous())
    if H == Ht:
        Bih, Bhh = mod._bias_views(li)
    else:
        Bih = c.get(("bih", li), bih, lambda: torch.cat([_pad_gate_rows(p.detach(), G, Ht, H) for p in bih], 0))
        Bhh = c.get(("bhh", li), bhh, lambda: torch.stack([_pad_gate_rows(p.detach(), G, Ht, H) for p in bhh], 0))
    sv, Xh = None, X
    if has_bn:
        bn = layer.batch_norm.module
        Xh = ops.empty_padded(R, I, X.dtype, X.device)
        sv = _bn_seq_fwd(bn, bn_w, bn_b, X, Xh, R, layer.input_size, I, training)
    if ops.split3_ok(dtype, R, D * G * H, I):
        Wih3 = c.get(("wih3", li), wih, lambda: ops.split3(Wih, 1))
        GI = ops.gemm_nt(ops.split3(Xh, 0), Wih3, bias=Bih, out_dtype=torch.float32, rows=rows)
    else:
        GI = ops.gemm_nt(Xh, Wih, bias=Bih, rows=rows)
    if H != Ht:
        h0 = _pad_cols(h0, H) if h0 is not None else None
        c0 = _pad_cols(c0, H) if c0 is not None else None
    hext, Sv, hn, cn = ops.rnn_fwd(kind, GI, Whh, Bhh, lens_dev, D, N, H, Tp, h0=h0, c0=c0)
    if H != Ht:
        hn = hn[..., :Ht].contiguous()
        cn = cn[..., :Ht].contiguous() if cn is not None else None
    del GI
    if D == 2:
        out = ops.add2(hext[0, 1:Tp + 1].reshape(R, H), hext[1, 1:Tp + 1].reshape(R, H))
    else:
        out = hext[0, 1:Tp + 1].reshape(R, H)
    return out, hn, cn, [X, Xh if has_bn else None, hext, Sv], (kind, H, D, G, I, has_bn, sv, Ht, layer.input_size)


def _rnn_layer_backward(mod, li, meta, saved, lparams, dout, lens_dev, N, Tp, dtype, main, side, rows=None, state=None):
    kind, H, D, G, I, has_bn, sv, Ht, It = meta
    if state is not None:
        h0, c0, want = state
        h0p = _pad_cols(h0, H) if (h0 is not None and H != Ht) else h0
        c0p = _pad_cols(c0, H) if (c0 is not None and H != Ht) else c0
        state = (h0p, c0p, bool(want))
    dX, grads, rg = _rnn_layer_backward_impl(mod, li, meta, saved, lparams, dout, lens_dev, N, Tp, dtype, main, side, rows, state)
    if state is None:
        return dX, grads, None
    main.wait_stream(side)
    GH, po = G * H, (2 if has_bn else 0)
    if h0p is not None:
        n4 = (N + 3) // 4 * 4
        ar = torch.arange(N, device=lens_dev.device)
        for d in range(D):
            t_first = torch.zeros_like(ar) if d == 0 else (lens_dev.long().clamp(1, Tp) - 1)
            src = rg.dGH[d].reshape(Tp * N, GH) if (kind == "gru" and rg.dGH is not None) else rg.dGI[:, d * GH:(d + 1) * GH]
            g_first = src.index_select(0, t_first * N + ar).float()
            A = torch.zeros((GH, n4), dtype=torch.float32, device=g_first.device)
            A[:, :N] = g_first.t()
            B = torch.zeros((H, n4), dtype=torch.float32, device=g_first.device)
            B[:, :N] = h0p[d].t()
            corr = ops.gemm_nt(A, B, out_dtype=torch.float32)
            grads[po + 4 * d + 1] = grads[po + 4 * d + 1] + _unpad_gate_rows(corr, G, Ht, H)[:, :Ht]
    dstate = None
    if want:
        dstate = (rg.dh0[..., :Ht].contiguous(), rg.dc0[..., :Ht].contiguous() if rg.dc0 is not None else None)
    return dX, grads, dstate


def _rnn_transposed_weights(mod, li, meta, lparams, dtype):
    kind, H, D, G, I, has_bn, sv, Ht, It = meta
    po = 2 if has_bn else 0
    wih = [lparams[po + 4 * d + 0] for d in range(D)]
    whh = [lparams[po + 4 * d + 1] for d in range(D)]
    WhhT = mod._cache.get(("whhT", li, dtype), whh, lambda: torch.stack(
        [_pad_gate_rows(_pad_cols(p.detach(), H), G, Ht, H).t() for p in whh], 0).to(dtype).contiguous())

    def build_ihT():
        w = torch.cat([_pad_gate_rows(p.detach(), G, Ht, H) for p in wih], 0)
        w = _perm_cols_to_internal(w) if li == 0 else _pad_cols(w, H)
        return w.t().to(dtype).contiguous()
    return WhhT, mod._cache.get(("wihT", li, dtype), wih, build_ihT)


def _wgrad_path(dtype, kind, R, D, GH, H, Xh, rg=None):
    if ops.wgrad_tn_ok(dtype, R, D * GH, Xh.shape[1], lda=D * GH, ldb=Xh.stride(0)) and \
            ops.wgrad_tn_ok(dtype, R, GH, H, lda=D * GH, ldb=H):
        return "tn"
    if rg is None:
        return None
    if ops.split3_ok(dtype, GH, H, R, leaf=True) and FP32_WGRAD_TN and Xh.shape[1] % 8 == 0 and \
            ops.wgrad_tn_ok(torch.bfloat16, 3 * R, D * GH, Xh.shape[1]) and ops.wgrad_tn_ok(torch.bfloat16, 3 * R, GH, H) and \
            (kind != "gru" or rg.dQ is not None or rg.dGH is not None):
        return "tn_split"
    return "nt"


def _rnn_layer_backward_impl(mod, li, meta, saved, lparams, dout, lens_dev, N, Tp, dtype, main, side, rows=None, state=None):
    kind, H, D, G, I, has_bn, sv, Ht, It = meta
    X, Xh, hext, Sv = saved
    if Xh is None:
        Xh = X
    R, GH = Tp * N, G * H
    grads = [None] * len(lparams)
    WhhT, WihT = _rnn_transposed_weights(mod, li, meta, lparams, dtype)
    path = _wgrad_path(dtype, kind, R, D, GH, H, Xh)
    n_probs = 1 + D * (2 if (kind == "gru" and (2 * H) % 256 != 0) else 1)
    fuse_dx = path == "tn" and WGRAD_WITH_DX and n_probs < 6 and WihT.dim() == 2 and WihT.data_ptr() % 16 == 0 and \
        ops.gemm8_nt_shape_ok(dtype, R, WihT.shape[0], D * GH, D * GH, WihT.stride(0))
    if state is None:
        rg = ops.rnn_bwd(kind, dout, WhhT, hext, Sv, lens_dev, D, N, H, Tp, pad_rows_unread=bool(fuse_dx and rows is not None))
    else:
        rg = ops.rnn_bwd(kind, dout, WhhT, hext, Sv, lens_dev, D, N, H, Tp, h0=state[0], c0=state[1], want_dstate=state[2])
    dGI = rg.dGI
    layer = (mod, li, meta, lparams, grads, Xh, hext, rg, N, Tp)
    if fuse_dx:
        dXh = _wgrad_tn(*layer, rows=rows, dx=(dGI, WihT), zero_pad=(lens_dev, Tp, N))
    else:
        if path == "tn":
            _wgrad_tn(*layer, rows=rows)
        if ops.split3_ok(dtype, R, H, GH):
            po = 2 if has_bn else 0
            WihT3 = mod._cache.get(("wihT3", li), [lparams[po + 4 * d] for d in range(D)], lambda: ops.split3(WihT, 1))
            dXh = ops.gemm_nt(ops.split3(dGI, 0), WihT3, out_dtype=torch.float32, rows=rows, zero_pad=(lens_dev, Tp, N))
        else:
            dXh = ops.gemm_nt(dGI, WihT, rows=rows, zero_pad=(lens_dev, Tp, N))
    if has_bn:
        dX = torch.empty_like(dXh)
        grads[0], grads[1] = _bn_seq_bwd(dXh, X, dX, sv, R, It, I)
    else:
        dX = dXh
    if path == "tn":
        return dX, grads, rg
    ready = torch.cuda.Event()
    ready.record(main)
    with torch.cuda.stream(side):
        side.wait_event(ready)
        for t in rg.tensors() + [Xh, hext]:
            t.record_stream(side)
        if _wgrad_path(dtype, kind, R, D, GH, H, Xh, rg) == "tn_split":
            _wgrad_tn(*layer, split=True)
        else:
            _wgrad_nt(*layer)
    return dX, grads, rg


def _h_prev(hext, d, Tp, R, H):
    return (hext[d, 0:Tp] if d == 0 else hext[d, 2:Tp + 2]).reshape(R, H)


def _wgrad_problems(kind, rg, Xh, hext, Tp, operand, two_block, dWih, dWhh):
    D, GH, H = dWhh.shape
    R = rg.dGI.shape[0]
    A, B = operand(rg.dGI, 0), operand(Xh, 1)
    lda = A.stride(0)
    probs = [dict(At=A, Bt=B, M=D * GH, N=Xh.shape[1], lda=lda, ldb=B.stride(0), out=dWih)]
    for d in range(D):
        Hp = operand(_h_prev(hext, d, Tp, R, H), 1)
        hh = dict(Bt=Hp, N=H, ldb=Hp.stride(0))
        if kind == "gru" and rg.dQ is not None:
            Q = operand(rg.dQ[d].reshape(R, H), 0)
            if two_block:
                probs.append(dict(hh, At=A[:, d * GH:], At2=Q, lda2=Q.stride(0), m_split=2 * H, M=GH, lda=lda, out=dWhh[d]))
            else:
                probs.append(dict(hh, At=A[:, d * GH:], M=2 * H, lda=lda, out=dWhh[d, :2 * H]))
                probs.append(dict(hh, At=Q, M=H, lda=Q.stride(0), out=dWhh[d, 2 * H:]))
        elif kind == "gru":
            Gd = operand(rg.dGH[d].reshape(R, GH), 0)
            probs.append(dict(hh, At=Gd, M=GH, lda=Gd.stride(0), out=dWhh[d]))
        else:
            probs.append(dict(hh, At=A[:, d * GH:], M=GH, lda=lda, out=dWhh[d]))
    return probs


def _rnn_bias_grads(kind, rg, D, N, H):
    R, GH = rg.dGI.shape[0], rg.dGI.shape[1] // D
    if rg.bacc is not None:
        dBih, dBhh_all = ops.rnn_bias_grads(kind, rg.bacc, D, N, H)
        return dBih, dBhh_all, [dBhh_all[d] for d in range(D)]
    dBih = ops.colsum(rg.dGI)
    if kind == "gru":
        return dBih, None, [ops.colsum(rg.dGH[d].reshape(R, GH)) for d in range(D)]
    return dBih, None, [dBih[d * GH:(d + 1) * GH] for d in range(D)]


def _deliver_layer_grads(mod, li, meta, lparams, grads, per_dir, own):
    kind, H, D, G, I, has_bn, sv, Ht, It = meta
    po = 2 if has_bn else 0
    for d in range(D):
        grads[po + 4 * d:po + 4 * d + 4] = per_dir[d]
    sync = getattr(mod, "_grad_sync", None)
    if sync is not None and H == Ht:
        sync.layer_ready(own, lparams[po:po + 4 * D])
    _unpad_layer_grads(grads, po, D, G, Ht, H, It, li == 0)


def _wgrad_tn(mod, li, meta, lparams, grads, Xh, hext, rg, N, Tp, split=False, rows=None, dx=None, zero_pad=None):
    kind, H, D, G = meta[:4]
    GH, dev = G * H, rg.dGI.device
    K = (3 if split else 1) * Tp * N
    dWih = torch.empty((D * GH, Xh.shape[1]), dtype=torch.float32, device=dev)
    dWhh = torch.empty((D, GH, H), dtype=torch.float32, device=dev)
    probs = _wgrad_problems(kind, rg, Xh, hext, Tp, ops.split3_rows if split else (lambda t, mode: t),
                            not split and (2 * H) % 256 == 0, dWih, dWhh)
    dXh = None
    if dx is not None:
        assert ops.gemm8_nt_ok(dx[0], dx[1], K, dx[1].shape[0], D * GH, D * GH, dx[1].stride(0))
        _, dXh = ops.gemm8_tn_grouped(probs, K, dx=dx, rows=rows, zero_pad=zero_pad)
    else:
        ops.gemm8_tn_grouped(probs, K, rows=rows)
    if li == 0:
        dWih = torch.cat([_perm_cols_to_reference(dWih[d * GH:(d + 1) * GH], mod._rnn_in) for d in range(D)], 0)
    dBih, dBhh_all, dBhh_l = _rnn_bias_grads(kind, rg, D, N, H)
    per_dir = [(dWih[d * GH:(d + 1) * GH], dWhh[d], dBih[d * GH:(d + 1) * GH], dBhh_l[d]) for d in range(D)]
    own = [dWih, dWhh, dBih] + ([dBhh_all] if dBhh_all is not None else dBhh_l if kind == "gru" else [])
    _deliver_layer_grads(mod, li, meta, lparams, grads, per_dir, own)
    return dXh


def _wgrad_nt(mod, li, meta, lparams, grads, Xh, hext, rg, N, Tp):
    kind, H, D, G = meta[:4]
    R, GH, dGI, cores = Tp * N, G * H, rg.dGI, li > 0
    s3 = ops.split3_ok(dGI.dtype, GH, H, R, leaf=True)
    dGI_T = ops.transpose(dGI)
    Xh_T = ops.transpose(Xh)
    ldT = dGI_T.shape[1]
    dGI_T3 = ops.split3(dGI_T, 0) if s3 else None
    if s3:
        dWih = ops.gemm_nt(dGI_T3, ops.split3(Xh_T, 1), out_dtype=torch.float32, coresident=cores)
    else:
        dWih = ops.gemm_nt(dGI_T, Xh_T, out_dtype=torch.float32, splitk=_wgrad_splitk(dGI_T.shape[0], Xh_T.shape[0], ldT),
                           coresident=cores)
    del Xh_T
    if li == 0:
        dWih = torch.cat([_perm_cols_to_reference(dWih[d * GH:(d + 1) * GH], mod._rnn_in) for d in range(D)], 0)
    bsum = None
    if rg.bacc is not None:
        bsum = [ops.colsum(rg.bacc[d]) for d in range(D)]
        dBih = torch.cat([b[:GH] for b in bsum], 0)
    else:
        dBih = ops.colsum(dGI)
    per_dir = []
    for d in range(D):
        Hp_T = ops.transpose(_h_prev(hext, d, Tp, R, H))
        if kind == "gru" and rg.dQ is not None:
            dQ_T = ops.transpose(rg.dQ[d].reshape(R, H))
            if s3:
                A3 = torch.empty((GH, 3 * ldT), dtype=torch.bfloat16, device=dGI.device)
                A3[:2 * H].copy_(dGI_T3[d * GH:d * GH + 2 * H])
                ops.split3(dQ_T, 0, out=A3[2 * H:])
                dWhh = ops.gemm_nt(A3, ops.split3(Hp_T, 1), out_dtype=torch.float32, coresident=cores)
            else:
                dWhh = ops.gemm_nt_rows2(dGI_T[d * GH:d * GH + 2 * H], dQ_T, 2 * H, Hp_T, GH, H, ldT, ldT, ldT,
                                         splitk=_wgrad_splitk(GH, H, ldT), coresident=cores)
            dBhh = torch.cat([bsum[d][:2 * H], bsum[d][3 * H:4 * H]], 0) if bsum is not None else \
                torch.cat([dBih[d * GH:d * GH + 2 * H], ops.colsum(rg.dQ[d].reshape(R, H))], 0)
        else:
            if kind == "gru":
                dGH_T = ops.transpose(rg.dGH[d].reshape(R, GH))
                dBhh = ops.colsum(rg.dGH[d].reshape(R, GH))
            else:
                dGH_T = dGI_T[d * GH:(d + 1) * GH]
                dBhh = dBih[d * GH:(d + 1) * GH]
            if s3:
# ... 677 lines not shown
```

deepspeech/pytorch_amd/ops.py:

```python
import ctypes as C

import numpy as np
import torch

from . import _lib
from ._lib import F32, BF16, call, query

CELLS = {"gru": _lib.CELL_GRU, "lstm": _lib.CELL_LSTM, "rnn": _lib.CELL_RNN_TANH}
GATES = {"gru": 3, "lstm": 4, "rnn": 1}
SAVED_PLANES = {"gru": 4, "lstm": 5, "rnn": 0}


def dt(t):
    d = t if isinstance(t, torch.dtype) else t.dtype
    if d == torch.float32:
        return F32
    if d == torch.bfloat16:
        return BF16
    raise TypeError("ds2hip supports float32 and bfloat16 activations, got %s" % d)


def vecw(dtype):
    return 4 if dtype == torch.float32 else 8

# ... 50 lines not shown
def empty_padded(rows, cols, dtype, device):
    ld = pad_ld(cols, dtype)
    return torch.empty((rows, ld), dtype=dtype, device=device)[:, :cols] if ld != cols else torch.empty((rows, cols), dtype=dtype, device=device)


GEMM8_ENABLED = True


def gemm8_nt_shape_ok(dtype, M, N, K, lda, ldb):
    return (GEMM8_ENABLED and dtype == torch.bfloat16 and K % 64 == 0 and lda % 8 == 0 and ldb % 8 == 0 and
            M >= 1024 and N >= 256 and rup(M, 256) // 256 * (rup(N, 256) // 256) >= 160 and M * lda < (1 << 31) and N * ldb < (1 << 31))


def gemm8_nt_ok(A, B, M, N, K, lda, ldb):
    return (A.dtype == B.dtype and gemm8_nt_shape_ok(A.dtype, M, N, K, lda, ldb) and
            A.data_ptr() % 16 == 0 and B.data_ptr() % 16 == 0)


def wgrad_tn_ok(dtype, R, M, N, lda=None, ldb=None):
    lda = M if lda is None else lda
    ldb = N if ldb is None else ldb
    return (GEMM8_ENABLED and dtype == torch.bfloat16 and R >= 512 and M % 8 == 0 and N % 8 == 0 and M >= 256 and N >= 256 and
            R * lda < (1 << 31) and R * ldb < (1 << 31))


def zero_pad_rows(X, lens, Tp, N):
    call("ds2_zero_pad_rows", dt(X), P(X), X.stride(0), X.shape[1], P(lens), Tp, N, S())
    return X


def gemm_nt(A, B, bias=None, out_dtype=None, M=None, N=None, K=None, lda=None, ldb=None, out=None, ldc=None, splitk=1,
            batch=1, sA=0, sB=0, sC=0, sBias=0, coresident=False, rows=None, zero_pad=None):
    M = A.shape[-2] if M is None else M
    N = B.shape[-2] if N is None else N
    K = A.shape[-1] if K is None else K
    lda = A.stride(-2) if lda is None else lda
    ldb = B.stride(-2) if ldb is None else ldb
    out_dtype = out_dtype or A.dtype
    if out is None and splitk == 1 and batch == 1 and not coresident and gemm8_nt_ok(A, B, M, N, K, lda, ldb):
        res = gemm8_nt(A, B, bias=bias, out_dtype=out_dtype, M=M, N=N, K=K, lda=lda, ldb=ldb, rows=rows)
        if rows is not None and zero_pad is not None:
            zero_pad_rows(res, *zero_pad)
        return res
    ks = fp32_ksplit(A.dtype, M, N, K) if (out is None and splitk == 1 and batch == 1 and not coresident and bias is None and
                                            out_dtype == torch.float32 and A.dtype == torch.float32) else 1
    if ks > 1:
        Ks = K // ks
        ws = torch.empty((ks, M, N), dtype=torch.float32, device=A.device)
        call("ds2_gemm_nt", dt(A), P(A), P(B), P(ws), None, M, N, Ks, lda, ldb, N, 1, ks, Ks, Ks, M * N, 0, 1, S())
        out = torch.empty((M, N), dtype=torch.float32, device=A.device)
        call("ds2_sum_slices", P(ws), P(out), M * N, ks, S())
        if rows is not None and zero_pad is not None:
            zero_pad_rows(out, *zero_pad)
        return out
    if out is None:
        shape = (batch, M, N) if batch > 1 else (M, N)
        out = torch.empty(shape, dtype=out_dtype, device=A.device)
        ldc = N
        sC = M * N
    out_f32 = 1 if out.dtype == torch.float32 else 0
    call("ds2_gemm_nt_coresident" if coresident else "ds2_gemm_nt", dt(A), P(A), P(B), P(out), PF(bias), M, N, K, lda, ldb, ldc,
         out_f32, batch, sA, sB, sC, sBias, splitk, S())
    if rows is not None and zero_pad is not None and batch == 1:
        zero_pad_rows(out, *zero_pad)
    return out


def kslice_plan(K, slices):
    nkt = K // 64
    for s_ in range(slices, max(1, slices // 2), -1):
        if nkt % s_ == 0 and K % 64 == 0:
            slices = s_
            break
    return slices, (K // max(slices, 1)) // 64 * 64


def head_kslices(R):
    return max(1, min(32, R // 2048))


def gemm_nt_kslices(A, B, slices):
    M, K = A.shape[-2], A.shape[-1]
    N = B.shape[-2]
    lda, ldb = A.stride(-2), B.stride(-2)
    slices, Ks = kslice_plan(K, slices)
    if slices <= 1 or Ks == 0 or (M * N) % 4 != 0:
        return gemm_nt(A, B, out_dtype=torch.float32)
    rest = K - slices * Ks
    ws = torch.empty((slices + (1 if rest else 0), M, N), dtype=torch.float32, device=A.device)
    call("ds2_gemm_nt", dt(A), P(A), P(B), P(ws), None, M, N, Ks, lda, ldb, N, 1, slices, Ks, Ks, M * N, 0, 1, S())
    if rest:
        call("ds2_gemm_nt", dt(A), P(A[:, slices * Ks:]), P(B[:, slices * Ks:]), P(ws[slices]), None, M, N, rest, lda, ldb, N, 1, 1,
             0, 0, 0, 0, 1, S())
    out = torch.empty((M, N), dtype=torch.float32, device=A.device)
    call("ds2_sum_slices", P(ws), P(out), M * N, ws.shape[0], S())
    return out


FC_CALLS = {"fwd": 0, "bwd": 0}


def fc_ok(dtype, H, Cp):
    return dtype == torch.bfloat16 and bool(query("ds2_fc_supported", int(H), int(Cp)))


def fc_fwd(Xh, Wp, R=None, H=None):
    R = Xh.shape[0] if R is None else R
    H = Wp.shape[1] if H is None else H
    Cp = Wp.shape[0]
    logits = torch.empty((R, Cp), dtype=torch.float32, device=Xh.device)
    call("ds2_fc_fwd", P(Xh), Xh.stride(0), P(Wp), Wp.stride(0), P(logits), Cp, R, H, Cp, S())
    FC_CALLS["fwd"] += 1
    return logits


def fc_bwd(dlogits, Xh, Wp, R=None, H=None):
    R = Xh.shape[0] if R is None else R
    H = Wp.shape[1] if H is None else H
    Cp = Wp.shape[0]
    dev = Xh.device
    K = rup(R, 64)
    slices, Ks = kslice_plan(K, head_kslices(R))
    block_rows = K if slices <= 1 or Ks == 0 else Ks
    dXh = torch.empty((R, H), dtype=torch.bfloat16, device=dev)
    dW = torch.empty((Cp, H), dtype=torch.float32, device=dev)
    ws = torch.empty((query("ds2_fc_bwd_partials", R, block_rows), Cp, H), dtype=torch.float32, device=dev)
    call("ds2_fc_bwd", PF(dlogits), dlogits.stride(0), P(Xh), Xh.stride(0), P(Wp), Wp.stride(0), P(dXh), H, P(dW), P(ws), R, H, Cp,
         block_rows, S())
    FC_CALLS["bwd"] += 1
    return dXh, dW


FP32_KSPLIT = __import__("os").environ.get("DS2_FP32_KSPLIT", "1") != "0"


def fp32_ksplit(dtype, M, N, K):
    if not FP32_KSPLIT or dtype != torch.float32 or K % 32 != 0 or (M * N) % 4 != 0:
        return 1
    tiles = ((M + 127) // 128) * ((N + 127) // 128)
    nkt = K // 32
    if tiles >= 128 or nkt < 32:
        return 1
    want = min(8, max(1, 256 // tiles))
    for s_ in range(want, 1, -1):
        if nkt % s_ == 0 and nkt // s_ >= 8:
            return s_
    return 1


def gemm_nt_rows2(A, A2, m_split, B, M, N, K, lda, ldb, splitk=1, coresident=False):
    out = torch.empty((M, N), dtype=torch.float32, device=A.device)
    call("ds2_gemm_nt_rows2", dt(A), P(A), P(A2), m_split, P(B), P(out), M, N, K, lda, ldb, N, 1, splitk, 1 if coresident else 0, S())
    return out


def gemm8_nt(A, B, bias=None, out_dtype=None, M=None, N=None, K=None, lda=None, ldb=None, rows=None):
    M = A.shape[-2] if M is None else M
    N = B.shape[-2] if N is None else N
    K = A.shape[-1] if K is None else K
    lda = A.stride(-2) if lda is None else lda
    ldb = B.stride(-2) if ldb is None else ldb
    out = torch.empty((M, N), dtype=out_dtype or A.dtype, device=A.device)
    if rows is not None:
        call("ds2_gemm8_nt_rows", P(A), P(B), P(out), PF(bias), M, N, K, lda, ldb, N, 1 if out.dtype == torch.float32 else 0, P(rows),
             rows.numel(), S())
        return out
    call("ds2_gemm8_nt", P(A), P(B), P(out), PF(bias), M, N, K, lda, ldb, N, 1 if out.dtype == torch.float32 else 0, S())
    return out


def gemm8_tn_grouped(problems, K, dx=None, rows=None, zero_pad=None):
    rp, nr = (P(rows), rows.numel()) if rows is not None else (None, 0)
    n = len(problems)
    outs = []
    for pr in problems:
        o = pr.get("out")
        if o is None:
            o = torch.empty((pr["M"], pr["N"]), dtype=torch.float32, device=pr["At"].device)
        outs.append(o)
    vp = C.c_void_p * n
    ia, la = C.c_int * n, C.c_long * n
    At = vp(*[pr["At"].data_ptr() for pr in problems])
    At2 = vp(*[(pr["At2"].data_ptr() if pr.get("At2") is not None else 0) for pr in problems])
    ms = ia(*[int(pr.get("m_split", 0)) for pr in problems])
    Bt = vp(*[pr["Bt"].data_ptr() for pr in problems])
    Cs = vp(*[o.data_ptr() for o in outs])
    Ms, Ns = ia(*[pr["M"] for pr in problems]), ia(*[pr["N"] for pr in problems])
    lda, ldb = la(*[pr["lda"] for pr in problems]), la(*[pr["ldb"] for pr in problems])
    lda2 = la(*[int(pr.get("lda2", 0)) for pr in problems])
    ldc = la(*[o.stride(0) for o in outs])
    for pr in problems:
        P(pr["At"]), P(pr["Bt"])
    if dx is not None:
        A, B = dx
        Mx, Nx, Kx = A.shape[0], B.shape[0], A.shape[1]
        out_x = torch.empty((Mx, Nx), dtype=A.dtype, device=A.device)
        call("ds2_gemm8_wgrad_dx_rows", n, At, At2, ms, Bt, Cs, Ms, Ns, lda, lda2, ldb, ldc, K, P(A), P(B), P(out_x), Mx, Nx, Kx, A.stride(0),
             B.stride(0), Nx, rp, nr, S())
        if rows is not None and zero_pad is not None:
            zero_pad_rows(out_x, *zero_pad)
        return outs, out_x
    call("ds2_gemm8_tn_grouped_rows", n, At, At2, ms, Bt, Cs, Ms, Ns, lda, lda2, ldb, ldc, K, rp, nr, S())
    return outs


def colsum(X, R=None, Cc=None, ld=None, scale=1.0):
    R = X.shape[0] if R is None else R
    Cc = X.shape[1] if Cc is None else Cc
    ld = X.stride(0) if ld is None else ld
    out = torch.empty(Cc, dtype=torch.float32, device=X.device)
    ws = torch.empty(query("ds2_norm_partials", R) * Cc, dtype=torch.float32, device=X.device)
    call("ds2_colsum", dt(X), P(X), R, Cc, ld, P(out), float(scale), P(ws), S())
    return out


import os as _os
FP32_GEMM_MODE = _os.environ.get("DS2_FP32_GEMM", "wgrad")
FP32_SPLIT3 = FP32_GEMM_MODE != "exact"


def split3_ok(dtype, M, N, K, leaf=False):
    if dtype != torch.float32 or FP32_GEMM_MODE == "exact" or not (M >= 256 and N >= 256 and K >= 256):
        return False
    return leaf or FP32_GEMM_MODE == "split3"


def split3(X, mode, out=None):
    rows, K = X.shape
    Kp = rup(K, 64)
    if out is None:
        out = torch.empty((rows, 3 * Kp), dtype=torch.bfloat16, device=X.device)
    assert out.shape[0] == rows and out.shape[1] == 3 * Kp and X.dtype == torch.float32 and X.stride(1) == 1
    call("ds2_split3_bf16", P(X), X.stride(0), rows, K, Kp, mode, P(out), out.stride(0), S())
    return out


def split3_rows(X, mode):
    rows, K = X.shape
    K8 = rup(K, 8)
    out = torch.empty((3 * rows, K8), dtype=torch.bfloat16, device=X.device)
    assert X.dtype == torch.float32 and X.stride(1) == 1
    call("ds2_split3_bf16", P(X), X.stride(0), rows, K, K8, 2 + mode, P(out), K8, S())
    return out


def transpose(X, R=None, Cc=None, lds=None):
    R = X.shape[0] if R is None else R
    Cc = X.shape[1] if Cc is None else Cc
    lds = X.stride(0) if lds is None else lds
    ldd = rup(R, 64)
    out = torch.empty((Cc, ldd), dtype=X.dtype, device=X.device)
    call("ds2_transpose", dt(X), P(X), P(out), R, Cc, lds, ldd, S())
    return out


def cast_transpose_bf16(src, dst=None, ldd=0, dstT=None, lddT=0, perm=None, cout=None):
    R, Cc = src.shape
    pc, pf = perm if perm is not None else (0, 0)
    call("ds2_cast_transpose_bf16", PF(src), src.stride(0), R, Cc, pc, pf, Cc if cout is None else cout,
         P(dst) if dst is not None else None, ldd, P(dstT) if dstT is not None else None, lddT, S())


def small_weight_layouts(w1, w2, wfc, dtype):
    dev, Cc, H = w1.device, wfc.shape[0], wfc.shape[1]
    w1k = torch.empty((451, 32), dtype=torch.float32, device=dev)
    w2t = torch.empty((21, 11, 32, 32), dtype=dtype, device=dev)
    w2d0 = torch.empty((11, 11, 32, 32), dtype=dtype, device=dev)
    w2d1 = torch.empty((10, 11, 32, 32), dtype=dtype, device=dev)
    wp = torch.empty((32, H), dtype=dtype, device=dev)
    wpT = torch.empty((H, 32), dtype=dtype, device=dev)
    call("ds2_small_weight_layouts", dt(dtype), PF(w1), PF(w2), PF(wfc), Cc, H, P(w1k), P(w2t), P(w2d0), P(w2d1), P(wp), P(wpT), S())
    return w1k, w2t, [w2d0, w2d1], wp, wpT


def scale_by_(x, s):
    call("ds2_scale_by", P(x), PF(s.reshape(1)), x.numel(), S())
    return x


def add2(a, b):
    out = torch.empty_like(a)
    call("ds2_add2", dt(a), P(a), P(b), P(out), a.numel(), S())
    return out


class BnSaved:
    __slots__ = ("mean", "rstd", "scale", "shift")

    def __init__(self, Cc, device):
        buf = torch.empty((4, Cc), dtype=torch.float32, device=device)
        self.mean, self.rstd, self.scale, self.shift = buf[0], buf[1], buf[2], buf[3]


def bn_fwd(X, mode, training, gamma, beta, rmean, rvar, nbt, R, Cc, ldx, Y, ldy, F=0, Tp=0, N=0, lens=None, eps=1e-5,
           momentum=0.1):
    sv = BnSaved(Cc, X.device)
    ws = torch.empty(2 * query("ds2_norm_partials", R) * Cc, dtype=torch.float32, device=X.device)
    call("ds2_bn_fwd", dt(X), mode, 1 if training else 0, P(X), P(Y), R, Cc, ldx, ldy, F, Tp, N, P(lens), PF(gamma), PF(beta),
         PF(rmean), PF(rvar), P(nbt) if training else C.c_void_p(0), float(eps), float(momentum), P(sv.mean), P(sv.rstd),
         P(sv.scale), P(sv.shift), P(ws), S())
    return sv


def bn_bwd(G, X, DX, mode, sv, R, Cc, ldg, ldx, lddx, F=0, Tp=0, N=0, lens=None):
    dgamma = torch.empty(Cc, dtype=torch.float32, device=X.device)
    dbeta = torch.empty(Cc, dtype=torch.float32, device=X.device)
    ws = torch.empty((2 * query("ds2_norm_partials", R) + 2) * Cc, dtype=torch.float32, device=X.device)
    call("ds2_bn_bwd", dt(X), mode, P(G), P(X), P(DX), R, Cc, ldg, ldx, lddx, F, Tp, N, P(lens), P(sv.mean), P(sv.rstd),
         P(sv.scale), P(sv.shift), P(dgamma), P(dbeta), P(ws), S())
    return dgamma, dbeta


def conv_rows(F0):
    F1 = (F0 + 2 * 20 - 41) // 2 + 1
    return F1, (F1 + 2 * 10 - 21) // 2 + 1


def conv1_fwd(x, w1k, b1, lens, Tp, dtype):
    N, _, F0, T = x.shape
    y1 = torch.empty((N, conv_rows(F0)[0], Tp, 32), dtype=dtype, device=x.device)
    call("ds2_conv1_fwd", dt(dtype), PF(x), PF(w1k), PF(b1), P(lens), P(y1), N, F0, T, Tp, S())
    return y1


def conv1_wgrad(x, dy1, Tp):
    N, _, F0, T = x.shape
    dw = torch.empty((451, 32), dtype=torch.float32, device=x.device)
    ws = torch.empty(query("ds2_conv1_wgrad_ws_floats", N, F0, Tp), dtype=torch.float32, device=x.device)
    call("ds2_conv1_wgrad", dt(dy1), P(x), P(dy1), P(dw), N, F0, T, Tp, P(ws), S())
    return dw


def conv2_fwd(a1, w2t, b2, lens, F0=161):
    N, F1, Tp, _ = a1.shape
    assert F1 == conv_rows(F0)[0]
    y2 = torch.empty((N, conv_rows(F0)[1], Tp, 32), dtype=a1.dtype, device=a1.device)
    nws = query("ds2_conv2_fwd_ws_bytes", dt(a1), N, F0, Tp)
    ws = torch.empty(nws, dtype=torch.uint8, device=a1.device) if nws else None
    call("ds2_conv2_fwd", dt(a1), P(a1), P(w2t), PF(b2), P(lens), P(y2), N, F0, Tp, P(ws), S())
    return y2


def conv2_dgrad(dy2, w2d_even, w2d_odd, F0=161):
    N, F2, Tp, _ = dy2.shape
    assert F2 == conv_rows(F0)[1]
    da1 = torch.empty((N, conv_rows(F0)[0], Tp, 32), dtype=dy2.dtype, device=dy2.device)
    call("ds2_conv2_dgrad", dt(dy2), P(dy2), P(w2d_even), P(w2d_odd), P(da1), N, F0, Tp, S())
    return da1


def conv2_wgrad(dy2, a1, F0=161):
    N, _, Tp, _ = dy2.shape
    dw = torch.empty((231, 32, 32), dtype=torch.float32, device=dy2.device)
    ws = torch.empty(query("ds2_conv2_wgrad_ws_floats", N, Tp), dtype=torch.float32, device=dy2.device)
    call("ds2_conv2_wgrad", dt(dy2), P(dy2), P(a1), P(dw), N, F0, Tp, P(ws), S())
    return dw


_PERSIST_ERR = {}
LAST_PERSIST_WS = None

STARTUP_MS_SINGLE = 300
STARTUP_MS_DP_MIN, STARTUP_MS_DP_MAX = 30_000, 3_600_000
_OPTS = {"variant": 0, "spin_limit": 0, "startup_ms": None}
FORCE_DATA_PARALLEL_BUDGET = [False]


class persist_options:

    def __init__(self, **kw):
        assert set(kw) <= set(_OPTS), kw
        self.kw = kw

    def __enter__(self):
        self.old = dict(_OPTS)
        _OPTS.update(self.kw)
        return self

    def __exit__(self, *exc):
        _OPTS.clear()
        _OPTS.update(self.old)
        return False


def data_parallel_ranks():
    try:
        import torch.distributed as _dist
        if _dist.is_available() and _dist.is_initialized():
            return int(_dist.get_world_size())
    except Exception:
        pass
    return 1


def persist_startup_ms():
    if _OPTS["startup_ms"] is not None:
        return int(_OPTS["startup_ms"])
    env = _os.environ.get("DS2_PERSIST_STARTUP_MS", "")
    if env:
        return max(1, int(env))
    if data_parallel_ranks() > 1 or FORCE_DATA_PARALLEL_BUDGET[0]:
        ms = 600_000
        try:
            import torch.distributed as _dist
            from torch.distributed.distributed_c10d import _get_default_group
            if _dist.is_initialized():
                to = getattr(_get_default_group(), "_timeout", None) or getattr(_dist, "default_pg_timeout", None)
                if to is not None:
                    ms = int(to.total_seconds() * 1000)
        except Exception:
            pass
        return min(max(ms, STARTUP_MS_DP_MIN), STARTUP_MS_DP_MAX)
    return STARTUP_MS_SINGLE


def _persist_opts():
    o = _lib.PersistOpts(int(_OPTS["variant"]), int(_OPTS["spin_limit"]), persist_startup_ms())
    return o


def persist_kind(dtype, kind, D, N, H):
    return query("ds2_rnn_persist_kind", dt(dtype), CELLS[kind], D, N, H, int(_OPTS["variant"]))


def _persist_err(dev):
    key = dev.index if dev.index is not None else torch.cuda.current_device()
    t = _PERSIST_ERR.get(key)
    if t is None:
        t = _PERSIST_ERR[key] = torch.zeros(16, dtype=torch.int32, device=dev)
    return t


def _persist_error_message(code, key):
    if code == 2:
        return ("a persistent recurrent sweep on device %d could not start: its workgroups never became co-resident within its start-up "
                "budget (%.1f s now; 0.3 s single-process, the process group's time-out under data parallelism, DS2_PERSIST_STARTUP_MS "
                "overrides) -- another kernel holds compute units (a second process on this GPU, e.g. a validation job or two ranks with "
                "the same LOCAL_RANK; or a long-running kernel on another stream).  The sweep gave up, its outputs were NaN-poisoned"
                % (key, persist_startup_ms() / 1000.0))
    return ("a persistent recurrent kernel timed out on device %d waiting for its peer workgroups in the middle of a sweep "
            "(are other kernels occupying CUs?); its outputs were NaN-poisoned" % key)


def check_persistent_kernels():
    for key, t in _PERSIST_ERR.items():
        code = int(t[0].item())
        if code != 0:
            raise _lib.Ds2HipError(_persist_error_message(code, key))


_ERR_MIRROR = {}


def poll_persistent_error(dev):
    key = dev.index if dev.index is not None else torch.cuda.current_device()
    t = _PERSIST_ERR.get(key)
    if t is None:
        return
    m = _ERR_MIRROR.get(key)
    if m is None:
        m = _ERR_MIRROR[key] = [torch.zeros(1, dtype=torch.int32).pin_memory(), None]
    if m[1] is not None:
        if not m[1].query():
            return
        m[1] = None
        if int(m[0][0]) != 0:
            raise _lib.Ds2HipError(_persist_error_message(int(m[0][0]), key))
    call("ds2_copy_words", P(t), C.c_void_p(m[0].data_ptr()), 1, S())
    ev = torch.cuda.Event()
    ev.record()
    m[1] = ev


class PinnedRing:

    def __init__(self, depth=32):
        self.depth = depth
        self._per_device = {}
        self._lock = __import__("threading").Lock()

    class _RingState:
        def __init__(self):
            self.cap, self.buf, self.events, self.i = 0, None, None, 0

    def stage(self, dev, parts):
        n = int(sum(p.size for p in parts))
        dev = torch.device(dev)
        if dev.type != "cuda":
            return torch.from_numpy(np.concatenate([np.asarray(p, dtype=np.int32).reshape(-1) for p in parts]) if parts else np.zeros(0, np.int32))
        key = dev.index if dev.index is not None else torch.cuda.current_device()
        with self._lock, torch.cuda.device(key):
            st = self._per_device.setdefault(key, PinnedRing._RingState())
            if st.buf is None or n > st.cap:
                if st.events is not None:
                    for e in st.events:
                        if e is not None:
                            e.synchronize()
                st.cap = max(1024, 1 << (max(n, 1) - 1).bit_length())
                st.buf = torch.empty(self.depth * st.cap, dtype=torch.int32, pin_memory=True)
                st.events = [None] * self.depth
                st.i = 0
            k = st.i
            st.i = (k + 1) % self.depth
            if st.events[k] is not None and not st.events[k].query():
                st.events[k].synchronize()
            slot = st.buf[k * st.cap:k * st.cap + n]
            hv = slot.numpy()
            o = 0
            for p in parts:
                hv[o:o + p.size] = np.asarray(p).reshape(-1)
                o += p.size
            out = torch.empty(n, dtype=torch.int32, device=torch.device("cuda", key))
            if n:
                dptr = _pinned_device_ptr(slot)
                if dptr is not None:
                    call("ds2_copy_words", C.c_void_p(dptr), P(out), n, S())
                else:
                    out.copy_(slot, non_blocking=True)
            if st.events[k] is None:
                st.events[k] = torch.cuda.Event()
            st.events[k].record()
            return out


_HIPRT = []


def _pinned_device_ptr(t):
    if not _HIPRT:
        try:
            lib = C.CDLL("libamdhip64.so")
            lib.hipHostGetDevicePointer.restype = C.c_int
            lib.hipHostGetDevicePointer.argtypes = [C.POINTER(C.c_void_p), C.c_void_p, C.c_uint]
            _HIPRT.append(lib)
        except OSError:
            _HIPRT.append(None)
    lib = _HIPRT[0]
    if lib is None:
        return t.data_ptr()
    dp = C.c_void_p(0)
    rc = lib.hipHostGetDevicePointer(C.byref(dp), C.c_void_p(t.data_ptr()), 0)
    return dp.value if rc == 0 and dp.value else None


POISON_UNWRITTEN = False
PERSIST_ENABLED = True


_WARNED_CUS = set()
_WARNED_SHAPES = set()
PERSIST_CLIFF_MIN_H = 256


def use_persistent(kind, dtype, D, N, H):
    if not PERSIST_ENABLED:
        return False
    ok = bool(query("ds2_rnn_persist_supported", dt(dtype), CELLS[kind], D, N, H, int(_OPTS["variant"])))
    if ok:
        return True
    import os
    import warnings
    covered = bool(query("ds2_rnn_persist_shape_covered", dt(dtype), CELLS[kind], D, N, H))
    if covered:
        dev = torch.cuda.current_device()
        cus = torch.cuda.get_device_properties(dev).multi_processor_count
        if os.environ.get("DS2_ALLOW_LAUNCH_PER_STEP", "0") in ("", "0"):
            raise _lib.Ds2HipError("ds2hip: device %d exposes %d compute units (< 256): the persistent recurrent kernels need one "
                                   "workgroup per CU, all co-resident.  Set DS2_ALLOW_LAUNCH_PER_STEP=1 to run the launch-per-time-step "
                                   "kernels instead (several times slower)." % (dev, cus))
        if dev not in _WARNED_CUS:
            _WARNED_CUS.add(dev)
            warnings.warn("ds2hip: device %d exposes %d compute units (< 256): the persistent recurrent kernels are disabled, the "
                          "recurrent sweeps use one launch per time step" % (dev, cus))
    elif H >= PERSIST_CLIFF_MIN_H:
        key = (kind, str(dtype), D, N, H)
        if key not in _WARNED_SHAPES:
            _WARNED_SHAPES.add(key)
            widths = [w for w in range(16, 2049, 16) if query("ds2_rnn_persist_shape_covered", dt(dtype), CELLS[kind], D, N, w)]
            warnings.warn("ds2hip: no persistent recurrent kernel is instantiated for %s %s hidden=%d, %d direction(s), batch %d: the "
                          "sweeps run one launch per time step (5-8x slower per step).  For this cell, type, direction count and batch "
                          "persistent kernels exist with hidden in {%s}; the model class zero-pads other hidden sizes up to the nearest "
                          "instantiated width when that is at most 1.5x as wide (DS2_PAD_HIDDEN)."
                          % (str(dtype).replace("torch.", ""), kind, H, D, N, ", ".join(map(str, widths))))
    return False


def rnn_fwd(kind, GI, Whh, bhh, lens, D, N, H, Tp, h0=None, c0=None, save=True):
    dev, dtype = GI.device, GI.dtype
    hext = torch.empty((D, Tp + 2, N, H), dtype=dtype, device=dev)
    persistent = use_persistent(kind, dtype, D, N, H)
    if not persistent:
        hext[:, 0].zero_()
        hext[:, Tp + 1].zero_()
    ns = SAVED_PLANES[kind]
    Sv = torch.empty((D, Tp, N, max(ns, 1) * H) if ns else (1,), dtype=dtype, device=dev)
    hn = torch.empty((D, N, H), dtype=torch.float32, device=dev)
    cn = torch.empty((D, N, H), dtype=torch.float32, device=dev) if kind == "lstm" else None
    if persistent:
        ws = torch.empty(query("ds2_rnn_persist_ws_bytes", dt(dtype), CELLS[kind], D, N, H, int(_OPTS["variant"])), dtype=torch.uint8, device=dev)
        global LAST_PERSIST_WS
        LAST_PERSIST_WS = ws
        po = _persist_opts()
        with _sweep_timer("rnn_fwd_persistent", Tp):
            call("ds2_rnn_persist_fwd", dt(dtype), CELLS[kind], D, N, H, Tp, P(lens), P(GI), P(Whh), PF(bhh), PF(h0), PF(c0),
                 P(hext[:, 1]), (Tp + 2) * N * H, P(Sv), P(hn), P(cn), P(ws), P(_persist_err(dev)), C.byref(po), S())
        return hext, Sv, hn, cn
    state = torch.empty(query("ds2_rnn_state_bytes", D, N, H), dtype=torch.uint8, device=dev)
    with _sweep_timer("rnn_fwd", Tp):
        call("ds2_rnn_fwd", dt(dtype), CELLS[kind], D, N, H, Tp, P(lens), P(GI), P(Whh), PF(bhh), PF(h0), PF(c0),
             P(hext[:, 1]), (Tp + 2) * N * H, P(Sv), P(hn), P(cn), P(state), S())
    return hext, Sv, hn, cn


class RnnGrads:
    __slots__ = ("dGI", "dGH", "dQ", "bacc", "dh0", "dc0")

    def __init__(self, dGI, dGH=None, dQ=None, bacc=None):
        self.dGI, self.dGH, self.dQ, self.bacc = dGI, dGH, dQ, bacc
        self.dh0 = self.dc0 = None

    def tensors(self):
        return [t for t in (self.dGI, self.dGH, self.dQ, self.bacc) if t is not None]


def rnn_bwd(kind, dOut, WhhT, hext, Sv, lens, D, N, H, Tp, pad_rows_unread=False, h0=None, c0=None, want_dstate=False):
    dev, dtype = dOut.device, dOut.dtype
    G = GATES[kind]
    dGI = torch.empty((Tp * N, D * G * H), dtype=dtype, device=dev)
    with_state = h0 is not None or c0 is not None or want_dstate
    if not with_state and use_persistent(kind, dtype, D, N, H):
        dQ = torch.empty((D, Tp, N, H), dtype=dtype, device=dev) if kind == "gru" else None
        if POISON_UNWRITTEN:
# ... 698 lines not shown
```

include/ds2hip.h:

```cpp
#ifndef DS2HIP_H
#define DS2HIP_H

#include <stdint.h>

#ifdef __cplusplus
extern "C" {
#endif

typedef void* ds2_stream_t;

enum { DS2_F32 = 0, DS2_BF16 = 1 };
enum { DS2_CELL_GRU = 0, DS2_CELL_LSTM = 1, DS2_CELL_RNN_TANH = 2 };
enum {
  DS2_OK = 0,
  DS2_ERR_DTYPE = 1001,
  DS2_ERR_ARG = 1002,
  DS2_ERR_ALIGN = 1003
};

int ds2_version(void);
const char* ds2_error_string(int code);

int ds2_gemm_nt(int dtype, const void* A, const void* B, void* C, const float* bias, int M, int N, int K, long lda, long ldb,
                long ldc, int out_f32, int batch, long strideA, long strideB, long strideC, long strideBias, int splitk,
                ds2_stream_t stream);

int ds2_gemm_nt_rows2(int dtype, const void* A, const void* A2, int m_split, const void* B, void* C, int M, int N, int K, long lda,
                      long ldb, long ldc, int out_f32, int splitk, int coresident, ds2_stream_t stream);
int ds2_gemm_nt_coresident(int dtype, const void* A, const void* B, void* C, const float* bias, int M, int N, int K, long lda,
                           long ldb, long ldc, int out_f32, int batch, long strideA, long strideB, long strideC, long strideBias,
                           int splitk, ds2_stream_t stream);

int ds2_gemm8_nt(const void* A, const void* B, void* C, const float* bias, int M, int N, int K, long lda, long ldb, long ldc, int out_f32,
                 ds2_stream_t stream);
int ds2_gemm8_tn_grouped(int n_problems, const void* const* At, const void* const* At2, const int* m_split, const void* const* Bt, void* const* C,
                         const int* M, const int* N, const long* lda, const long* lda2, const long* ldb, const long* ldc, int K, ds2_stream_t stream);

int ds2_gemm8_wgrad_dx(int n_tn, const void* const* At, const void* const* At2, const int* m_split, const void* const* Bt, void* const* C,
                       const int* M, const int* N, const long* lda, const long* lda2, const long* ldb, const long* ldc, int K_tn,
                       const void* A_nt, const void* B_nt, void* C_nt, int M_nt, int N_nt, int K_nt, long lda_nt, long ldb_nt, long ldc_nt,
                       ds2_stream_t stream);

int ds2_gemm8_nt_rows(const void* A, const void* B, void* C, const float* bias, int n_phys, int N, int K, long lda, long ldb, long ldc,
                      int out_f32, const int* rows, int n_rows, ds2_stream_t stream);
int ds2_gemm8_tn_grouped_rows(int n_problems, const void* const* At, const void* const* At2, const int* m_split, const void* const* Bt,
                              void* const* C, const int* M, const int* N, const long* lda, const long* lda2, const long* ldb, const long* ldc,
                              int n_phys, const int* rows, int n_rows, ds2_stream_t stream);
int ds2_gemm8_wgrad_dx_rows(int n_tn, const void* const* At, const void* const* At2, const int* m_split, const void* const* Bt, void* const* C,
                            const int* M, const int* N, const long* lda, const long* lda2, const long* ldb, const long* ldc, int K_tn,
                            const void* A_nt, const void* B_nt, void* C_nt, int M_nt, int N_nt, int K_nt, long lda_nt, long ldb_nt, long ldc_nt,
                            const int* rows, int n_rows, ds2_stream_t stream);
int ds2_zero_pad_rows(int dtype, void* X, long ld, int cols, const int* lens, int Tp, int N, ds2_stream_t stream);

int ds2_norm_partials(long R);
int ds2_bn_fwd(int dtype, int mode, int training, const void* X, void* Y, long R, int C, long ldx, long ldy, int F, int Tp,
               int N, const int* lens, const float* gamma, const float* beta, float* running_mean, float* running_var,
               long long* num_batches_tracked, float eps, float momentum, float* save_mean, float* save_rstd,
               float* save_scale, float* save_shift, float* ws, ds2_stream_t stream);
int ds2_bn_bwd(int dtype, int mode, const void* G, const void* X, void* DX, long R, int C, long ldg, long ldx, long lddx,
               int F, int Tp, int N, const int* lens, const float* save_mean, const float* save_rstd,
               const float* save_scale, const float* save_shift, float* dgamma, float* dbeta, float* ws,
               ds2_stream_t stream);
int ds2_colsum(int dtype, const void* X, long R, int C, long ld, float* out, float scale, float* ws, ds2_stream_t stream);

int ds2_conv_rows(int F0, int* F1, int* F2);
int ds2_conv1_fwd(int dtype, const float* x, const float* w1k, const float* b1, const int* lens, void* y1, int N, int F0, int T,
                  int Tp, ds2_stream_t stream);
long ds2_conv1_wgrad_ws_floats(int N, int F0, int Tp);
int ds2_conv1_wgrad(int dtype, const float* x, const void* dy1, float* dw1k, int N, int F0, int T, int Tp, float* ws,
                    ds2_stream_t stream);
long ds2_conv2_fwd_ws_bytes(int dtype, int N, int F0, int Tp);
int ds2_conv2_fwd(int dtype, const void* a1, const void* w2t, const float* b2, const int* lens, void* y2, int N, int F0, int Tp,
                  void* ws, ds2_stream_t stream);
int ds2_conv2_dgrad(int dtype, const void* dy2, const void* w2d_even, const void* w2d_odd, void* da1, int N, int F0, int Tp,
                    ds2_stream_t stream);
long ds2_conv2_wgrad_ws_floats(int N, int Tp);
int ds2_conv2_wgrad(int dtype, const void* dy2, const void* a1, float* dw2t, int N, int F0, int Tp, float* ws, ds2_stream_t stream);

int ds2_rnn_gates(int cell);
int ds2_rnn_saved_planes(int cell);
long ds2_rnn_state_bytes(int D, int N, int H);
int ds2_rnn_fwd(int dtype, int cell, int D, int N, int H, int Tp, const int* lens, const void* GI, const void* Whh,
                const float* bhh, const float* h0, const float* c0, void* Hseq, long hseq_dstride, void* S, float* hn, float* cn,
                void* state, ds2_stream_t stream);
int ds2_rnn_bwd(int dtype, int cell, int D, int N, int H, int Tp, const int* lens, const void* dOut, const void* WhhT,
                const void* Hseq, long hseq_dstride, const void* S, void* dGI, void* dGH, const float* h0, const float* c0,
                float* dh0, float* dc0, void* state, ds2_stream_t stream);

typedef struct ds2_persist_opts {
  unsigned variant;
  unsigned spin_limit;
  unsigned startup_ms;
} ds2_persist_opts;
int ds2_rnn_persist_plan(int dtype, int cell, int D, int N, int H, int cus, unsigned variant, long* ws_bytes);
int ds2_rnn_persist_supported(int dtype, int cell, int D, int N, int H, unsigned variant);
int ds2_rnn_persist_shape_covered(int dtype, int cell, int D, int N, int H);
int ds2_rnn_persist_kind(int dtype, int cell, int D, int N, int H, unsigned variant);
long ds2_rnn_persist_ws_bytes(int dtype, int cell, int D, int N, int H, unsigned variant);
int ds2_rnn_persist_fwd(int dtype, int cell, int D, int N, int H, int Tp, const int* lens, const void* GI, const void* Whh,
                        const float* bhh, const float* h0, const float* c0, void* Hseq, long hseq_dstride, void* S, float* hn,
                        float* cn, void* ws, int* err, const ds2_persist_opts* opts, ds2_stream_t stream);
int ds2_rnn_persist_bwd(int dtype, int cell, int D, int N, int H, int Tp, const int* lens, const void* dOut, const void* WhhT,
                        const void* Hseq, long hseq_dstride, const void* S, void* dGI, void* dQ, float* dBacc, int flags, void* ws,
                        int* err, const ds2_persist_opts* opts, ds2_stream_t stream);

int ds2_add2(int dtype, const void* a, const void* b, void* out, long n, ds2_stream_t stream);
int ds2_sum_slices(const float* src, float* out, long n, int slices, ds2_stream_t stream);
int ds2_transpose(int dtype, const void* src, void* dst, long R, int C, long lds, long ldd, ds2_stream_t stream);
int ds2_split3_bf16(const float* src, long lds, long rows, int K, int Kp, int mode, void* dst, long ldd, ds2_stream_t stream);
int ds2_cast_transpose_bf16(const float* src, long lds, int R, int C, int perm_c, int perm_f, int Cout, void* dst, long ldd,
                            void* dstT, long lddT, ds2_stream_t stream);
int ds2_small_weight_layouts(int dtype, const float* w1, const float* w2, const float* wfc, int C, int H, float* w1k, void* w2t,
                             void* w2d0, void* w2d1, void* wfcp, void* wfcT, ds2_stream_t stream);
int ds2_scale_by(float* x, const float* s, long n, ds2_stream_t stream);

int ds2_copy_words(const void* src, void* dst, long n_words, ds2_stream_t stream);
int ds2_lookahead_fwd(int dtype, const void* x, const float* w, void* y, void* pre, int Tp, int N, int H, int ctx,
                      ds2_stream_t stream);
long ds2_lookahead_ws_floats(int Tp, int N, int H, int ctx);
int ds2_lookahead_bwd(int dtype, const void* x, const float* w, const void* pre, const void* dy, void* dx, float* dw, int Tp,
                      int N, int H, int ctx, float* ws, ds2_stream_t stream);
int ds2_rnn_bias_grads(int cell, int D, int N, int H, const float* dBacc, float* dbih, float* dbhh, ds2_stream_t stream);

int ds2_fc_supported(int H, int Cp);
int ds2_fc_fwd(const void* Xh, long ldx, const void* Wp, long ldw, float* logits, long ldl, long R, int H, int Cp, ds2_stream_t stream);
long ds2_fc_bwd_partials(long R, long block_rows);
int ds2_fc_bwd(const float* dlogits, long ldg, const void* Xh, long ldx, const void* Wp, long ldw, void* dXh, long lddx, float* dW,
               float* ws, long R, int H, int Cp, long block_rows, ds2_stream_t stream);

int ds2_softmax_rows(const float* logits, float* probs, long rows, int C, long ld_in, long ld_out, ds2_stream_t stream);

long ds2_ctc_ws_floats(int Tp, int N, int C, int max_target_len);
int ds2_ctc_loss_grad(const float* logits, long ldl, const int* targets, const int* target_offsets, const int* input_lengths,
                      const int* target_lengths, int Tp, int N, int C, int blank, int max_target_len, float grad_scale,
                      float* nll, float* loss_sum, float* dlogits, long ldg, float* ws, int recursion, ds2_stream_t stream);

int ds2_opt_max_tensors(void);
long ds2_clip_ws_floats(int count, const long* n);
int ds2_clip_coef(int count, const float* const* g, const long* n, float max_norm, float* out, float* ws, ds2_stream_t stream);
int ds2_opt_multi(int mode, int count, float* const* p, const float* const* g, float* const* m, float* const* v, const long* n,
                  const float* hp, int first, const float* clip, ds2_stream_t stream);
int ds2_opt_matrix(int mode, float* p, const float* g, float* m, float* v, int R, int C, int perm_c, int perm_f, int Cout,
                   void* dst, long ldd, void* dstT, long lddT, const float* hp, int first, const float* clip, ds2_stream_t stream);
int ds2_opt_matrices(int mode, int count, float* const* p, const float* const* g, float* const* m, float* const* v, const int* R,
                     const int* C, const int* perm_c, const int* perm_f, const int* Cout, void* const* dst, const long* ldd,
                     void* const* dstT, const long* lddT, const float* hp, int first, const float* clip, ds2_stream_t stream);

int ds2_spect_frames(int nsamples);
long ds2_spect_ws_bytes(int N, int Lmax);
int ds2_spectrogram(const float* wav, long ldw, const int* nsamples, int N, int Lmax, const float* basis, int reflect,
                    int normalize, float* out, void* ws, ds2_stream_t stream);

int ds2_spectrogram_aug(const float* wav, long ldw, const int* nsamples, int N, int Lmax, const float* basis, int reflect,
                        int normalize, float* out, void* ws, const float* warp_draw, int W, const int* fmask, int MF,
                        const int* tmask, int MT, float* coef_out, ds2_stream_t stream);
int ds2_spec_augment_coef(const float* x, int N, int F, int Tmax, const int* frames, const float* warp_draw, int W, float* coef,
                          ds2_stream_t stream);
int ds2_spec_augment(const float* in, float* out, int N, int F, int Tmax, const int* frames, const float* coef, const int* fmask,
                     int MF, const int* tmask, int MT, ds2_stream_t stream);

int ds2_wsola_segments(int nsamples, float tempo);
long ds2_wsola_out_len(int nsamples, float tempo);
int ds2_wsola(const float* wav, long ldw, const int* nsamples, const float* tempo, int N, float* out, long ldo, int* nsamples_out,
              int* offsets, int Smax, ds2_stream_t stream);
long ds2_wave_ws_bytes(int N);
int ds2_wave_energy(const float* wav, long ldw, const int* nsamples, int N, const float* gain, const float* level,
                    const float* bank, long bank_len, const long long* noise_off, const int* noise_start, void* ws,
                    ds2_stream_t stream);
int ds2_wave_mix(const float* wav, long ldw, const int* nsamples, int N, const float* gain, const float* level, const float* bank,
                 long bank_len, const long long* noise_off, const int* noise_start, const void* ws, float* out, long ldo,
                 ds2_stream_t stream);

int ds2_greedy_decode(const float* x, long stride_n, long stride_t, int N, int T, int C, const int* sizes, int blank,
                      int* tokens, int* offsets, int* counts, ds2_stream_t stream);

int ds2_greedy_stream_feed(const float* x, long stride_n, long stride_t, int N, int Tc, int C, const int* sizes, int blank,
                           int* carry, int* tokens, int* offsets, int* counts, ds2_stream_t stream);

long ds2_beam_ws_bytes(int N, int T, int B);
int ds2_beam_decode(const float* x, long stride_n, long stride_t, int N, int T, int C, const int* sizes, int blank, int B,
                    int cutoff_top_n, float cutoff_prob, int* tokens, int* offsets, int* lens, float* scores, void* ws,
                    ds2_stream_t stream);

int ds2_beam_decode_lm(const float* x, long stride_n, long stride_t, int N, int T, int C, const int* sizes, int blank, int B,
                       int cutoff_top_n, float cutoff_prob, int space, const void* word_table, long word_slots,
                       const void* ngram_table, long ngram_slots, int order, int bos, float alpha, float beta, int lexicon,
                       int* tokens, int* offsets, int* lens, float* scores, float* acoustic, void* ws, ds2_stream_t stream);

long ds2_beam_grid_ws_bytes(int G, int N, int T, int B);
int ds2_beam_decode_lm_grid(const float* x, long stride_n, long stride_t, int N, int T, int C, const int* sizes, int blank, int B,
                            int cutoff_top_n, float cutoff_prob, int space, const void* word_table, long word_slots,
                            const void* ngram_table, long ngram_slots, int order, int bos, int lexicon, int G, const float* alphas,
                            const float* betas, int* tokens, int* offsets, int* lens, float* scores, float* acoustic, void* ws,
                            ds2_stream_t stream);

long ds2_beam_stream_bytes(int N, int B, int max_frames, int lm);
long ds2_beam_stream_ws_bytes(int N, int Tc);
long ds2_beam_stream_state_stride(int B, int lm);
int ds2_beam_stream_reset(void* state, int N, int B, int max_frames, int lm, const int* mask, ds2_stream_t stream);
int ds2_beam_stream_feed(const float* x, long stride_n, long stride_t, int N, int Tc, int C, const int* sizes, int blank, int B,
                         int cutoff_top_n, float cutoff_prob, void* state, int max_frames, int* tokens, int* offsets,
                         long row_stride, int out_ranks, int* lens, float* scores, void* ws, ds2_stream_t stream);
int ds2_beam_stream_feed_lm(const float* x, long stride_n, long stride_t, int N, int Tc, int C, const int* sizes, int blank, int B,
                            int cutoff_top_n, float cutoff_prob, int space, const void* word_table, long word_slots,
                            const void* ngram_table, long ngram_slots, int order, int bos, float alpha, float beta, int lexicon,
                            void* state, int max_frames, int* tokens, int* offsets, long row_stride, int out_ranks, int* lens,
                            float* scores, float* acoustic, void* ws, ds2_stream_t stream);

int ds2_stream_plan(long frames, int chunk, int ctx, int final, int* out);
long ds2_stream_state_bytes(int dtype, int N, int F0, int H, int ctx);
int ds2_stream_conv1(int dtype, const float* x, const float* carry, float* next, const float* w1k, const float* b1,
                     const float* scale, const float* shift, const int* len, const int* live, void* y, int N, int F0, int Tc,
                     int off, int J, ds2_stream_t stream);
int ds2_stream_conv2(int dtype, const void* a1, const void* carry, void* next, const void* w2t, const float* b2, const float* scale,
                     const float* shift, const int* len, const int* live, void* x0, int N, int F0, int Jin, int off, int J,
                     int rld, ds2_stream_t stream);
int ds2_stream_lookahead(int dtype, const void* x, const void* carry, void* next, const float* w, const int* len, void* y, int N,
                         int H, int ctx, int Jin, int off, int J, ds2_stream_t stream);

typedef struct ds2_stream_row {
  int32_t slot;
  int32_t src;
  int32_t cur;
  int32_t fresh;
  int32_t len;
  int32_t off1, cnt1;
  int32_t off2, cnt2;
  int32_t off3, cnt3;
  int32_t reserved[5];
} ds2_stream_row;
int ds2_stream_conv1_rows(int dtype, const float* x, float* carry0, float* carry1, const ds2_stream_row* rows, const float* w1k,
                          const float* b1, const float* scale, const float* shift, void* y, int n_rows, int F0, int Tc, int J,
                          ds2_stream_t stream);
int ds2_stream_conv2_rows(int dtype, const void* a1, void* carry0, void* carry1, const ds2_stream_row* rows, const void* w2t,
                          const float* b2, const float* scale, const float* shift, void* x0, int n_rows, int n_rnn, int F0, int Jin,
                          int J, int rld, ds2_stream_t stream);
int ds2_stream_lookahead_rows(int dtype, const void* x, void* carry0, void* carry1, const ds2_stream_row* rows, const float* w, void* y,
                              int n_rnn, int S, int H, int ctx, int Jin, int J, ds2_stream_t stream);

int ds2_error_counts(const int* hyp, long hyp_stride, const int* hyp_lens, int P, const int* ref, const int* ref_offsets, int R,
                     int space, int* char_err, int* word_err, int* ref_chars, int* ref_words, ds2_stream_t stream);

long ds2_ctc_align_ws_bytes(int Tp, int N, int max_target_len);
int ds2_ctc_align(const float* x, long stride_n, long stride_t, int N, int Tp, int C, int mode, const int* sizes, const int* targets,
                  const int* target_offsets, const int* target_lengths, int max_target_len, int blank, int* frame_state,
                  int* tok_start, int* tok_end, float* tok_logp, float* score, void* ws, ds2_stream_t stream);

#ifdef __cplusplus
}
#endif
#endif
```

Measured before the change: 21730.

## Stage conv1 input as padded bf16 image with LDS-DMA kernels; fuse bias grads into BN bwd

Adds a pre-pass that writes the conv1 input as a zero-padded bf16 image. New persistent forward and weight-gradient conv1 kernels stream tiles from that image into LDS with buffer-load-to-LDS, double-buffered, feeding MFMA. This replaces per-element fp32 gathers with boundary checks. Separately, the conv bias gradients are computed inside the batch-norm backward pass, dropping two separate column-sum passes over dy1 and dy2. In exchange it costs an extra image-conversion kernel, extra memory kept for backward, and complex hand-scheduled code.

```diff
diff --git a/deepspeech/pytorch_amd/_lib.py b/deepspeech/pytorch_amd/_lib.py
--- a/deepspeech/pytorch_amd/_lib.py
+++ b/deepspeech/pytorch_amd/_lib.py
@@ -26,11 +26,16 @@
     "ds2_bn_fwd": (_i, [_i, _i, _i, _vp, _vp, _l, _i, _l, _l, _i, _i, _i, _vp, _vp, _vp, _vp, _vp, _vp, _f, _f, _vp, _vp,
                         _vp, _vp, _vp, _vp]),
     "ds2_bn_bwd": (_i, [_i, _i, _vp, _vp, _vp, _l, _i, _l, _l, _l, _i, _i, _i, _vp, _vp, _vp, _vp, _vp, _vp, _vp, _vp, _vp]),
+    "ds2_bn_bwd_bias": (_i, [_i, _i, _vp, _vp, _vp, _l, _i, _l, _l, _l, _i, _i, _i, _vp, _vp, _vp, _vp, _vp, _vp, _vp, _vp, _vp, _vp]),
     "ds2_colsum": (_i, [_i, _vp, _l, _i, _l, _vp, _f, _vp, _vp]),
     "ds2_conv_rows": (_i, [_i, _vp, _vp]),
     "ds2_conv1_fwd": (_i, [_i, _vp, _vp, _vp, _vp, _vp, _i, _i, _i, _i, _vp]),
     "ds2_conv1_wgrad_ws_floats": (_l, [_i, _i, _i]),
     "ds2_conv1_wgrad": (_i, [_i, _vp, _vp, _vp, _i, _i, _i, _i, _vp, _vp]),
+    "ds2_conv1_image_bytes": (_l, [_i, _i, _i]),
+    "ds2_conv1_image": (_i, [_vp, _vp, _i, _i, _i, _vp]),
+    "ds2_conv1_fwd_img": (_i, [_vp, _vp, _vp, _vp, _vp, _i, _i, _i, _vp]),
+    "ds2_conv1_wgrad_img": (_i, [_vp, _vp, _vp, _i, _i, _i, _vp, _vp]),
     "ds2_conv2_fwd_ws_bytes": (_l, [_i, _i, _i, _i]),
     "ds2_conv2_fwd": (_i, [_i, _vp, _vp, _vp, _vp, _vp, _i, _i, _i, _vp, _vp]),
     "ds2_conv2_dgrad": (_i, [_i, _vp, _vp, _vp, _vp, _i, _i, _i, _vp]),
diff --git a/deepspeech/pytorch_amd/csrc/ds2_conv.hip b/deepspeech/pytorch_amd/csrc/ds2_conv.hip
--- a/deepspeech/pytorch_amd/csrc/ds2_conv.hip
+++ b/deepspeech/pytorch_amd/csrc/ds2_conv.hip
@@ -978,6 +978,336 @@
   return conv_tap_launch_nt<T, 1>(a, st);
 }
 
+constexpr int M1I_PADF = 20, M1I_LEAD = 5;
+constexpr int M1I_ROWS = F0 + 2 * M1I_PADF;
+constexpr int M1_CPR = M1_RSB / 16;
+constexpr int M1_CHUNKS = M1_PR * M1_CPR;
+constexpr int M1_PIECES = (M1_CHUNKS + 63) / 64;
+constexpr int M1_PPW = (M1_PIECES + 3) / 4;
+constexpr int M1_BUF = M1_PIECES * 1024;
+static_assert(M1_PATCH_BYTES % 16 == 0 && M1_BUF >= M1_PATCH_BYTES && M1_RSB % 16 == 0, "a patch is whole 16-byte chunks");
+
+__global__ void __launch_bounds__(256) k_conv1_image(const float* __restrict__ x, bf16_t* __restrict__ xb, int T, int pitch) {
+  const int c8 = blockIdx.x * 256 + threadIdx.x;
+  if (c8 * 8 >= pitch) return;
+  const int r = blockIdx.y, n = blockIdx.z, fi = r - M1I_PADF, t0 = c8 * 8 - M1I_LEAD;
+  uint4 o = make_uint4(0u, 0u, 0u, 0u);
+  if (fi >= 0 && fi < F0 && t0 + 7 >= 0 && t0 < T) {
+    const float* xr = x + ((long)n * F0 + fi) * T;
+    float v[8];
+#pragma unroll
+    for (int e = 0; e < 8; ++e) v[e] = xr[min(max(t0 + e, 0), T - 1)];
+#pragma unroll
+    for (int e = 0; e < 8; ++e) v[e] = (unsigned)(t0 + e) < (unsigned)T ? v[e] : 0.f;
+    o = make_uint4(cvt_pk_bf16(v[0], v[1]), cvt_pk_bf16(v[2], v[3]), cvt_pk_bf16(v[4], v[5]), cvt_pk_bf16(v[6], v[7]));
+  }
+  *reinterpret_cast<uint4*>(xb + ((long)n * M1I_ROWS + r) * pitch + c8 * 8) = o;
+}
+
+struct M1Next {
+  __amdgpu_buffer_rsrc_t rx;
+  int wave;
+  int voff[M1_PPW];
+};
+__device__ __forceinline__ void m1_next_init(M1Next& nx, const bf16_t* xb, long image_bytes, int pitch, int wave, int lane) {
+  nx.rx = __builtin_amdgcn_make_buffer_rsrc((void*)xb, 0, (int)image_bytes, 0x00020000);
+  nx.wave = wave;
+#pragma unroll
+  for (int i = 0; i < M1_PPW; ++i) {
+    const int c = 64 * (wave + 4 * i) + lane, pr = c / M1_CPR;
+    nx.voff[i] = c < M1_CHUNKS ? pr * (pitch * 2) + (c - pr * M1_CPR) * 16 : CW_OOB;
+  }
+}
+__device__ __forceinline__ void m1_dma_tile(const M1Next& nx, unsigned char* patch, int n, int tb, int fb, int pitch) {
+  const int soff = __builtin_amdgcn_readfirstlane(((n * M1I_ROWS + 18 * fb) * pitch + 256 * tb) * 2);
+#pragma unroll
+  for (int i = 0; i < M1_PPW; ++i) {
+    const int p = nx.wave + 4 * i;
+    if (4 * i + 3 < M1_PIECES || p < M1_PIECES)
+      __builtin_amdgcn_raw_ptr_buffer_load_lds(nx.rx, (cw_lds_ptr_t)(patch + p * 1024), 16, nx.voff[i], soff, 0, 0);
+  }
+}
+#define M1_WAIT_VM0() asm volatile("s_waitcnt vmcnt(0)" ::: "memory")
+#define M1_WAIT_LGKM(n) asm volatile("s_waitcnt lgkmcnt(" #n ")" ::: "memory")
+__device__ __forceinline__ void m1_publish() {
+  M1_WAIT_VM0();
+  __builtin_amdgcn_sched_barrier(0);
+  __builtin_amdgcn_s_barrier();
+  __builtin_amdgcn_sched_barrier(0);
+}
+
+#define M1_RD2(dst, addr, d0) asm volatile("ds_read2_b32 %0, %1 offset0:%2 offset1:%3" : "=v"(dst) : "v"(addr), "i"(d0), "i"((d0) + 1))
+constexpr int M1F_AH = 2;
+struct M1Frag {
+  uint2 lo, hi;
+};
+template <int RHO>
+__device__ __forceinline__ void m1f_read(M1Frag (&bq)[M1F_AH + 1], uint32_t a0) {
+  const uint32_t a = a0 + (RHO / 2) * (2 * M1_RSB);
+  constexpr int d = (RHO & 1) * (M1_RSB / 4);
+  M1_RD2(bq[RHO % (M1F_AH + 1)].lo, a, d);
+  M1_RD2(bq[RHO % (M1F_AH + 1)].hi, a, d + 2);
+}
+struct M1Out {
+  uint2 o[M1_FB][4];
+  bf16_t* dst;
+  long rstride;
+};
+constexpr int M1F_ST0 = 3;
+template <int K>
+__device__ __forceinline__ void m1f_store(const M1Out& po) {
+  if (po.dst) *reinterpret_cast<uint2*>(po.dst + (K / 4) * po.rstride + 8 * (K % 4)) = po.o[K / 4][K % 4];
+}
+template <int K>
+__device__ __forceinline__ void m1f_store_all(const M1Out& po) {
+  m1f_store<K>(po);
+  if constexpr (K + 1 < 4 * M1_FB) m1f_store_all<K + 1>(po);
+}
+template <int RHO>
+__device__ __forceinline__ void m1f_row(ds2_f32x16 (&acc)[M1_FB], const uint4 (&A)[K1F], M1Frag (&bq)[M1F_AH + 1], uint32_t a0,
+                                        const M1Out& po) {
+  if constexpr (RHO + M1F_AH < M1_PR) m1f_read<RHO + M1F_AH>(bq, a0);
+  constexpr int left = M1F_AH < M1_PR - 1 - RHO ? M1F_AH : M1_PR - 1 - RHO;
+  static_assert(M1F_AH == 2, "the waits below are spelled for two rows ahead");
+  if constexpr (left == 2) M1_WAIT_LGKM(4);
+  else if constexpr (left == 1) M1_WAIT_LGKM(2);
+  else M1_WAIT_LGKM(0);
+  __builtin_amdgcn_sched_barrier(0);
+  const M1Frag& f = bq[RHO % (M1F_AH + 1)];
+  const uint4 b = make_uint4(f.lo.x, f.lo.y, f.hi.x, f.hi.y);
+#pragma unroll
+  for (int fl = 0; fl < M1_FB; ++fl) {
+    const int kf = RHO - 2 * fl;
+    if (kf >= 0 && kf < K1F) Mma<bf16_t>::mma32(acc[fl], A[kf], b);
+  }
+  if constexpr (RHO >= M1F_ST0 && RHO < M1F_ST0 + 4 * M1_FB) m1f_store<RHO - M1F_ST0>(po);
+  __builtin_amdgcn_sched_barrier(0);
+  if constexpr (RHO + 1 < M1_PR) m1f_row<RHO + 1>(acc, A, bq, a0, po);
+}
+static_assert(M1F_ST0 + 4 * M1_FB <= M1_PR, "every pending store has a row");
+
+__global__ void __launch_bounds__(256, 1) k_conv1_fwd_img(const bf16_t* __restrict__ xb, const float* __restrict__ w1k,
+                                                          const float* __restrict__ b1, const int* __restrict__ lens,
+                                                          bf16_t* __restrict__ y1, int N, int Tp, int ntb, int pitch, long image_bytes) {
+  __shared__ __attribute__((aligned(16))) unsigned char patch[2 * M1_BUF];
+  const int tid = threadIdx.x, lane = tid & 63, wave = __builtin_amdgcn_readfirstlane(tid >> 6);
+  const int pos = lane & 31, h = lane >> 5;
+  uint4 A[K1F];
+#pragma unroll
+  for (int kf = 0; kf < K1F; ++kf) {
+    float v[8];
+#pragma unroll
+    for (int i = 0; i < 8; ++i) {
+      const int kt = 8 * h + i;
+      const float wv = w1k[(kf * K1T + min(kt, K1T - 1)) * CH + pos];
+      v[i] = kt < K1T ? wv : 0.f;
+    }
+    A[kf] = make_uint4(cvt_pk_bf16(v[0], v[1]), cvt_pk_bf16(v[2], v[3]), cvt_pk_bf16(v[4], v[5]), cvt_pk_bf16(v[6], v[7]));
+  }
+#ifndef M1F_APIN
+#define M1F_APIN 17
+#endif
+#pragma unroll
+  for (int kf = K1F - M1F_APIN; kf < K1F; ++kf) {
+    typedef __attribute__((ext_vector_type(4))) unsigned int u4v;
+    u4v v = __builtin_bit_cast(u4v, A[kf]);
+    asm volatile("" : "+a"(v));
+    A[kf] = __builtin_bit_cast(uint4, v);
+  }
+  float bias[16];
+#pragma unroll
+  for (int r = 0; r < 16; ++r) bias[r] = b1[mma32_row(r, lane)];
+  const uint32_t lds0 = (uint32_t)(uintptr_t)(__attribute__((address_space(3))) unsigned char*)patch;
+  const uint32_t bp = lds0 + wave * 128 + pos * 4 + h * 16;
+  M1Next nx;
+  m1_next_init(nx, xb, image_bytes, pitch, wave, lane);
+  M1Out po;
+  po.dst = nullptr;
+  po.rstride = (long)Tp * CH;
+#pragma unroll
+  for (int fl = 0; fl < M1_FB; ++fl)
+#pragma unroll
+    for (int g = 0; g < 4; ++g) po.o[fl][g] = make_uint2(0u, 0u);
+  const int total = N * ntb * 9;
+  int blk = blockIdx.x;
+  if (blk < total) m1_dma_tile(nx, patch, blk / (9 * ntb), (blk / 9) % ntb, blk % 9, pitch);
+  m1_publish();
+  for (int buf = 0; blk < total; blk += gridDim.x, buf ^= 1) {
+    const int fb = blk % 9, tb = (blk / 9) % ntb, n = blk / (9 * ntb);
+    const int next = blk + gridDim.x;
+    if (next < total) m1_dma_tile(nx, patch + (buf ^ 1) * M1_BUF, next / (9 * ntb), (next / 9) % ntb, next % 9, pitch);
+    const int len = lens[n];
+    ds2_f32x16 acc[M1_FB];
+#pragma unroll
+    for (int fl = 0; fl < M1_FB; ++fl)
+#pragma unroll
+      for (int r = 0; r < 16; ++r) acc[fl][r] = bias[r];
+    const int tw = tb * M1_TB + wave * 32;
+    if (tw < min(len, Tp)) {
+      M1Frag bq[M1F_AH + 1];
+      const uint32_t a0 = bp + buf * M1_BUF;
+      M1_WAIT_LGKM(0);
+      __builtin_amdgcn_sched_barrier(0);
+      m1f_read<0>(bq, a0);
+      m1f_read<1>(bq, a0);
+      m1f_row<0>(acc, A, bq, a0, po);
+    } else {
+      m1f_store_all<0>(po);
+    }
+    const int t = tw + pos;
+    const bool live = t < len;
+    po.dst = t < Tp ? y1 + (((long)n * F1 + 9 * fb) * Tp + t) * CH + 4 * h : nullptr;
+#pragma unroll
+    for (int fl = 0; fl < M1_FB; ++fl)
+#pragma unroll
+      for (int g = 0; g < 4; ++g) {
+        const uint2 o = make_uint2(cvt_pk_bf16(acc[fl][4 * g], acc[fl][4 * g + 1]), cvt_pk_bf16(acc[fl][4 * g + 2], acc[fl][4 * g + 3]));
+        po.o[fl][g] = live ? o : make_uint2(0u, 0u);
+      }
+    m1_publish();
+  }
+  m1f_store_all<0>(po);
+}
+
+constexpr int M1WI_SMEM = 2 * M1_BUF + 4 * M1_DYT_WAVE;
+static_assert(K1F * K1T * CH * 4 <= M1WI_SMEM, "reduction buffer aliases the staging area");
+constexpr int M1W_AH = 3, M1W_NIT = 2 * M1_PR;
+struct M1Taps {
+  uint2 d[4];
+};
+template <int IT>
+__device__ __forceinline__ void m1w_taps(M1Taps (&xq)[M1W_AH + 1], uint32_t a0) {
+  constexpr int rho = IT >> 1, c = IT & 1;
+  const uint32_t a = a0 + (rho / 2) * (2 * M1_RSB);
+  constexpr int d = (rho & 1) * (M1_RSB / 4) + c * 32;
+  M1Taps& x = xq[IT % (M1W_AH + 1)];
+  M1_RD2(x.d[0], a, d);
+  M1_RD2(x.d[1], a, d + 2);
+  M1_RD2(x.d[2], a, d + 4);
+  M1_RD2(x.d[3], a, d + 6);
+}
+template <int IT>
+__device__ __forceinline__ void m1w_step(ds2_f32x4 (&acc)[K1F], const uint4 (&dyb)[M1_FB][2], M1Taps (&xq)[M1W_AH + 1], uint32_t a0,
+                                         uint32_t sel) {
+  constexpr int rho = IT >> 1, c = IT & 1;
+  if constexpr (IT + M1W_AH < M1W_NIT) m1w_taps<IT + M1W_AH>(xq, a0);
+  constexpr int left = M1W_AH < M1W_NIT - 1 - IT ? M1W_AH : M1W_NIT - 1 - IT;
+  static_assert(M1W_AH == 3, "the waits below are spelled for three operands ahead");
+  if constexpr (left == 3) M1_WAIT_LGKM(12);
+  else if constexpr (left == 2) M1_WAIT_LGKM(8);
+  else if constexpr (left == 1) M1_WAIT_LGKM(4);
+  else M1_WAIT_LGKM(0);
+  __builtin_amdgcn_sched_barrier(0);
+  const M1Taps& x = xq[IT % (M1W_AH + 1)];
+  const uint4 xa = make_uint4(__builtin_amdgcn_perm(x.d[0].y, x.d[0].x, sel), __builtin_amdgcn_perm(x.d[1].y, x.d[1].x, sel),
+                              __builtin_amdgcn_perm(x.d[2].y, x.d[2].x, sel), __builtin_amdgcn_perm(x.d[3].y, x.d[3].x, sel));
+#pragma unroll
+  for (int fl = 0; fl < M1_FB; ++fl) {
+    const int kf = rho - 2 * fl;
+    if (kf >= 0 && kf < K1F) Mma<bf16_t>::mma16(acc[kf], xa, dyb[fl][c]);
+  }
+  __builtin_amdgcn_sched_barrier(0);
+  if constexpr (IT + 1 < M1W_NIT) m1w_step<IT + 1>(acc, dyb, xq, a0, sel);
+}
+
+__global__ void __launch_bounds__(256, 1) k_conv1_wgrad_img(const bf16_t* __restrict__ xb, const bf16_t* __restrict__ dy1,
+                                                            float* __restrict__ partial, int N, int Tp, int ntb, int pitch,
+                                                            long image_bytes) {
+  extern __shared__ __attribute__((aligned(16))) unsigned char smem1i[];
+  const int tid = threadIdx.x, lane = tid & 63, wave = __builtin_amdgcn_readfirstlane(tid >> 6);
+  const int pair = wave >> 1, hh = wave & 1;
+  uint16_t* dyT = reinterpret_cast<uint16_t*>(smem1i + 2 * M1_BUF + wave * M1_DYT_WAVE);
+  const int kt = lane & 15, q = lane >> 4;
+  ds2_f32x4 acc[K1F];
+#pragma unroll
+  for (int kf = 0; kf < K1F; ++kf) acc[kf] = ds2_f32x4{0.f, 0.f, 0.f, 0.f};
+  const uint32_t lds0 = (uint32_t)(uintptr_t)(__attribute__((address_space(3))) unsigned char*)smem1i;
+  const uint32_t xp = lds0 + (2 * (64 * pair + 8 * q) + (kt & ~1)) * 2;
+  const uint32_t sel = (kt & 1) ? 0x07060302u : 0x05040100u;
+  M1Next nx;
+  m1_next_init(nx, xb, image_bytes, pitch, wave, lane);
+  const int total = N * ntb * 9;
+  const int piece = lane & 1;
+  uint4 dv[M1_FB][2];
+  auto load_dy = [&](int b) {
+    const int fb = b % 9, tb = (b / 9) % ntb, n = b / (9 * ntb);
+    const int t0 = tb * M1_TB + 64 * pair;
+#pragma unroll
+    for (int fl = 0; fl < M1_FB; ++fl)
+#pragma unroll
+      for (int j = 0; j < 2; ++j) {
+        const int t = t0 + 32 * j + (lane >> 1);
+        const uint4 v = *reinterpret_cast<const uint4*>(dy1 + (((long)n * F1 + 9 * fb + fl) * Tp + min(t, Tp - 1)) * CH + 16 * hh + 8 * piece);
+        dv[fl][j] = t < Tp ? v : make_uint4(0u, 0u, 0u, 0u);
+      }
+  };
+  int blk = blockIdx.x;
+  if (blk < total) {
+    m1_dma_tile(nx, smem1i, blk / (9 * ntb), (blk / 9) % ntb, blk % 9, pitch);
+    load_dy(blk);
+  }
+  m1_publish();
+  for (int buf = 0; blk < total; blk += gridDim.x, buf ^= 1) {
+#pragma unroll
+    for (int fl = 0; fl < M1_FB; ++fl)
+#pragma unroll
+      for (int j = 0; j < 2; ++j) {
+        const int tl = 32 * j + (lane >> 1);
+        const uint4 v = dv[fl][j];
+        uint16_t* d = dyT + (fl * 16 + 8 * piece) * M1_DYS + tl;
+        d[0 * M1_DYS] = (uint16_t)v.x;
+        d[1 * M1_DYS] = (uint16_t)(v.x >> 16);
+        d[2 * M1_DYS] = (uint16_t)v.y;
+        d[3 * M1_DYS] = (uint16_t)(v.y >> 16);
+        d[4 * M1_DYS] = (uint16_t)v.z;
+        d[5 * M1_DYS] = (uint16_t)(v.z >> 16);
+        d[6 * M1_DYS] = (uint16_t)v.w;
+        d[7 * M1_DYS] = (uint16_t)(v.w >> 16);
+      }
+    uint4 dyb[M1_FB][2];
+#pragma unroll
+    for (int fl = 0; fl < M1_FB; ++fl)
+#pragma unroll
+      for (int c = 0; c < 2; ++c) dyb[fl][c] = *reinterpret_cast<const uint4*>(dyT + (fl * 16 + kt) * M1_DYS + 32 * c + 8 * q);
+    M1_WAIT_LGKM(0);
+    __builtin_amdgcn_sched_barrier(0);
+    const int next = blk + gridDim.x;
+    if (next < total) {
+      m1_dma_tile(nx, smem1i + (buf ^ 1) * M1_BUF, next / (9 * ntb), (next / 9) % ntb, next % 9, pitch);
+      load_dy(next);
+    }
+    __builtin_amdgcn_sched_barrier(0);
+    {
+      M1Taps xq[M1W_AH + 1];
+      const uint32_t a0 = xp + buf * M1_BUF;
+      m1w_taps<0>(xq, a0);
+      m1w_taps<1>(xq, a0);
+      m1w_taps<2>(xq, a0);
+      m1w_step<0>(acc, dyb, xq, a0, sel);
+    }
+    m1_publish();
+  }
+  float* red = reinterpret_cast<float*>(smem1i);
+  for (int w = 0; w < 2; ++w) {
+    __syncthreads();
+    if (pair == w) {
+#pragma unroll
+      for (int kf = 0; kf < K1F; ++kf)
+#pragma unroll
+        for (int r = 0; r < 4; ++r) {
+          const int k = 4 * q + r;
+          if (k < K1T) {
+            float* e = red + (kf * K1T + k) * CH + 16 * hh + kt;
+            *e = w == 0 ? acc[kf][r] : *e + acc[kf][r];
+          }
+        }
+    }
+  }
+  __syncthreads();
+  float* dst = partial + (long)blockIdx.x * (K1F * K1T * CH);
+  for (int e = tid; e < K1F * K1T * CH; e += 256) dst[e] = red[e];
+}
+
 }
 
 static bool conv_geometry(int f0, int& f1, int& f2) {
@@ -1057,6 +1387,59 @@
   return ds2_colsum(DS2_F32, ws, P, C, C, dw1k, 1.0f, ws + (long)P * C, st_);
 }
 
+static int conv1_image_pitch(int Tp) { return 2 * M1_TB * ds2_cdiv(Tp, M1_TB) + 16; }
+static bool conv1_image_geometry(int N, int F0_, int T, int& Tp, int& pitch, long& bytes) {
+  if (N <= 0 || T <= 0 || F0_ != F0) return false;
+  Tp = (T + 2 * 5 - 10 - 1) / 2 + 1;
+  pitch = conv1_image_pitch(Tp);
+  bytes = (long)N * M1I_ROWS * pitch * 2;
+  return true;
+}
+long ds2_conv1_image_bytes(int N, int F0_, int T) {
+  int Tp, pitch;
+  long bytes;
+  return conv1_image_geometry(N, F0_, T, Tp, pitch, bytes) ? bytes : 0;
+}
+int ds2_conv1_image(const float* x, void* xb, int N, int F0_, int T, ds2_stream_t st_) {
+  hipStream_t st = (hipStream_t)st_;
+  int Tp, pitch;
+  long bytes;
+  DS2_REQUIRE(conv1_image_geometry(N, F0_, T, Tp, pitch, bytes) && N <= 65535, DS2_ERR_ARG);
+  hipLaunchKernelGGL(k_conv1_image, dim3(ds2_cdiv(pitch / 8, 256), M1I_ROWS, N), dim3(256), 0, st, x, (bf16_t*)xb, T, pitch);
+  DS2_CHECK_LAUNCH();
+  return 0;
+}
+int ds2_conv1_fwd_img(const void* xb, const float* w1k, const float* b1, const int* lens, void* y1, int N, int T, int Tp,
+                      ds2_stream_t st_) {
+  hipStream_t st = (hipStream_t)st_;
+  int tp, pitch;
+  long bytes;
+  DS2_REQUIRE(conv1_image_geometry(N, F0, T, tp, pitch, bytes) && tp == Tp && bytes < (long)CW_OOB, DS2_ERR_ARG);
+  const int ntb = ds2_cdiv(Tp, M1_TB);
+  const long total = (long)N * ntb * 9;
+  const int cus = ds2_cu_count();
+  hipLaunchKernelGGL(k_conv1_fwd_img, dim3((unsigned)(total < cus ? total : cus)), dim3(256), 0, st, (const bf16_t*)xb, w1k, b1, lens,
+                     (bf16_t*)y1, N, Tp, ntb, pitch, bytes);
+  DS2_CHECK_LAUNCH();
+  return 0;
+}
+int ds2_conv1_wgrad_img(const void* xb, const void* dy1, float* dw1k, int N, int T, int Tp, float* ws, ds2_stream_t st_) {
+  hipStream_t st = (hipStream_t)st_;
+  int tp, pitch;
+  long bytes;
+  DS2_REQUIRE(conv1_image_geometry(N, F0, T, tp, pitch, bytes) && tp == Tp && bytes < (long)CW_OOB, DS2_ERR_ARG);
+  int P = conv1_wgrad_blocks(N, F1, Tp);
+  static bool attr[DS2_MAX_DEVICES];
+  if (ds2_first_use_on_device(attr))
+    (void)hipFuncSetAttribute((const void*)k_conv1_wgrad_img, hipFuncAttributeMaxDynamicSharedMemorySize, M1WI_SMEM);
+  P = conv1_wgrad_mfma_blocks(N, Tp) < P ? conv1_wgrad_mfma_blocks(N, Tp) : P;
+  hipLaunchKernelGGL(k_conv1_wgrad_img, dim3(P), dim3(256), M1WI_SMEM, st, (const bf16_t*)xb, (const bf16_t*)dy1, ws, N, Tp,
+                     ds2_cdiv(Tp, M1_TB), pitch, bytes);
+  DS2_CHECK_LAUNCH();
+  const int C = K1F * K1T * CH;
+  return ds2_colsum(DS2_F32, ws, P, C, C, dw1k, 1.0f, ws + (long)P * C, st_);
+}
+
 long ds2_conv2_fwd_ws_bytes(int dtype, int N, int F0_, int Tp) { return (dtype == DS2_BF16 && F0_ == F0) ? (long)N * F2 * Tp * CH * 4 : 0; }
 int ds2_conv2_fwd(int dtype, const void* a1, const void* w2t, const float* b2, const int* lens, void* y2, int N, int F0_, int Tp, void* ws,
                   ds2_stream_t st_) {
diff --git a/deepspeech/pytorch_amd/csrc/ds2_norm.hip b/deepspeech/pytorch_amd/csrc/ds2_norm.hip
--- a/deepspeech/pytorch_amd/csrc/ds2_norm.hip
+++ b/deepspeech/pytorch_amd/csrc/ds2_norm.hip
@@ -284,16 +284,40 @@
   c2[c] = (float)(q / count);
 }
 
-template <typename T, bool CONV, bool SEQ_IN>
+template <typename T>
+__device__ __forceinline__ void store_and_keep(T* p, float (&o)[Vec16<T>::N]);
+template <>
+__device__ __forceinline__ void store_and_keep<float>(float* p, float (&o)[4]) {
+  Vec16<float>::store(p, o);
+}
+template <>
+__device__ __forceinline__ void store_and_keep<bf16_t>(bf16_t* p, float (&o)[8]) {
+  uint32_t w[4];
+#pragma unroll
+  for (int i = 0; i < 4; ++i) w[i] = cvt_pk_bf16(o[2 * i], o[2 * i + 1]);
+  *reinterpret_cast<uint4*>(p) = make_uint4(w[0], w[1], w[2], w[3]);
+#pragma unroll
+  for (int i = 0; i < 4; ++i) {
+    o[2 * i] = __uint_as_float(w[i] << 16);
+    o[2 * i + 1] = __uint_as_float(w[i] & 0xffff0000u);
+  }
+}
+
+template <typename T, bool CONV, bool SEQ_IN, bool SUMS = false>
 __global__ void __launch_bounds__(NORM_RY* NORM_CX)
     k_bn_bwd_apply_cols(const T* __restrict__ G, const T* __restrict__ X, T* __restrict__ DX, long R, int C, long ldg, long ldx,
                         long lddx, const float* __restrict__ scale, const float* __restrict__ shift,
                         const float* __restrict__ mean, const float* __restrict__ rstd, const float* __restrict__ c1,
-                        const float* __restrict__ c2, RowMap rm, const int* __restrict__ lens, int N) {
+                        const float* __restrict__ c2, RowMap rm, const int* __restrict__ lens, int N,
+                        float* __restrict__ psum_dx = nullptr) {
   constexpr int V = Vec16<T>::N;
   const RedMap m(C / V);
-  if (!m.ok) return;
-  const int c0 = m.chunk * V;
+  if (!SUMS && !m.ok) return;
+  if (!m.ok) R = 0;
+  float bs[V];
+#pragma unroll
+  for (int i = 0; i < V; ++i) bs[i] = 0.f;
+  const int c0 = m.ok ? m.chunk * V : 0;
   float sc[V], sh[V], mu[V], rs[V], k1[V], k2[V];
 #pragma unroll
   for (int i = 0; i < V; ++i) {
@@ -333,7 +357,13 @@
         o[i] = bn_dx(gi, xh, sc[i], k1[i], k2[i]);
       }
     }
-    Vec16<T>::store(DX + r * lddx + c0, o);
+    if (SUMS) {
+      store_and_keep<T>(DX + r * lddx + c0, o);
+#pragma unroll
+      for (int i = 0; i < V; ++i) bs[i] += o[i];
+    } else {
+      Vec16<T>::store(DX + r * lddx + c0, o);
+    }
   };
   long r = m.first_row();
   for (; r + step < R; r += 2 * step) {
@@ -357,6 +387,15 @@
     Vec16<T>::load(X + r * ldx + c0, x0);
     Vec16<T>::load(g0p, g0);
     finish(r, t0, l0, x0, g0);
+  }
+  if (SUMS) {
+    __shared__ float red[NORM_RY][NORM_CX * V + 1];
+    float o[V];
+    red_block<V>(red, m, bs, o);
+    if (threadIdx.y == 0 && m.rsub == 0 && m.ok) {
+#pragma unroll
+      for (int i = 0; i < V; ++i) psum_dx[(long)blockIdx.y * C + (long)m.chunk * V + i] = o[i];
+    }
   }
 }
 
@@ -460,12 +499,14 @@
   return 0;
 }
 
-int ds2_bn_bwd(int dtype, int mode, const void* G, const void* X, void* DX, long R, int C, long ldg, long ldx, long lddx,
-               int F, int Tp, int N, const int* lens, const float* save_mean, const float* save_rstd,
-               const float* save_scale, const float* save_shift, float* dgamma, float* dbeta, float* ws, ds2_stream_t st_) {
+int ds2_bn_bwd_bias(int dtype, int mode, const void* G, const void* X, void* DX, long R, int C, long ldg, long ldx, long lddx,
+                    int F, int Tp, int N, const int* lens, const float* save_mean, const float* save_rstd,
+                    const float* save_scale, const float* save_shift, float* dgamma, float* dbeta, float* dbias, float* ws,
+                    ds2_stream_t st_) {
   hipStream_t st = (hipStream_t)st_;
   DS2_REQUIRE(dtype == DS2_F32 || dtype == DS2_BF16, DS2_ERR_DTYPE);
   DS2_REQUIRE(mode >= 0 && mode <= 2, DS2_ERR_ARG);
+  DS2_REQUIRE(dbias == nullptr || mode != 0, DS2_ERR_ARG);
   DS2_REQUIRE(mode == 0 || R < (1L << 31), DS2_ERR_ARG);
   const int V = dtype == DS2_F32 ? 4 : 8;
   DS2_REQUIRE(C % V == 0 && ldx % V == 0 && ldg % V == 0 && lddx % V == 0, DS2_ERR_ALIGN);
@@ -487,6 +528,9 @@
 #define LAUNCH_APP(TT, CV, SI)                                                                                          \
   hipLaunchKernelGGL((k_bn_bwd_apply_cols<TT, CV, SI>), agrd, blk, 0, st, (const TT*)G, (const TT*)X, (TT*)DX, R, C, ldg, \
                      ldx, lddx, save_scale, save_shift, save_mean, save_rstd, c1, c2, rm, lens, N)
+#define LAUNCH_APP_SUMS(TT, CV, SI)                                                                                           \
+  hipLaunchKernelGGL((k_bn_bwd_apply_cols<TT, true, SI, true>), grd, blk, 0, st, (const TT*)G, (const TT*)X, (TT*)DX, R, C, ldg, \
+                     ldx, lddx, save_scale, save_shift, save_mean, save_rstd, c1, c2, rm, lens, N, ps)
 #define BOTH(WHICH)                                        \
   if (dtype == DS2_F32) {                                  \
     if (mode == 0) WHICH(float, false, false);             \
@@ -502,12 +546,33 @@
   hipLaunchKernelGGL(k_bn_bwd_finalize, dim3(ds2_cdiv(C, FIN_COLS)), dim3(256), 0, st, ps, pq, P, C, (double)R, dgamma, dbeta,
                      c1, c2);
   DS2_CHECK_LAUNCH();
-  BOTH(LAUNCH_APP)
-  DS2_CHECK_LAUNCH();
+  if (dbias == nullptr) {
+    BOTH(LAUNCH_APP)
+    DS2_CHECK_LAUNCH();
+  } else {
+    if (dtype == DS2_F32) {
+      if (mode == 1) LAUNCH_APP_SUMS(float, true, false);
+      else LAUNCH_APP_SUMS(float, true, true);
+    } else {
+      if (mode == 1) LAUNCH_APP_SUMS(bf16_t, true, false);
+      else LAUNCH_APP_SUMS(bf16_t, true, true);
+    }
+    DS2_CHECK_LAUNCH();
+    hipLaunchKernelGGL(k_colsum_finalize, dim3(ds2_cdiv(C, FIN_COLS)), dim3(256), 0, st, ps, P, C, dbias, 1.0f);
+    DS2_CHECK_LAUNCH();
+  }
 #undef BOTH
 #undef LAUNCH_RED
 #undef LAUNCH_APP
+#undef LAUNCH_APP_SUMS
   return 0;
 }
 
-}
+int ds2_bn_bwd(int dtype, int mode, const void* G, const void* X, void* DX, long R, int C, long ldg, long ldx, long lddx,
+               int F, int Tp, int N, const int* lens, const float* save_mean, const float* save_rstd,
+               const float* save_scale, const float* save_shift, float* dgamma, float* dbeta, float* ws, ds2_stream_t st_) {
+  return ds2_bn_bwd_bias(dtype, mode, G, X, DX, R, C, ldg, ldx, lddx, F, Tp, N, lens, save_mean, save_rstd, save_scale, save_shift,
+                         dgamma, dbeta, nullptr, ws, st_);
+}
+
+}
diff --git a/deepspeech/pytorch_amd/model.py b/deepspeech/pytorch_amd/model.py
--- a/deepspeech/pytorch_amd/model.py
+++ b/deepspeech/pytorch_amd/model.py
@@ -261,7 +261,11 @@
         if x.shape[2] != F0:
             raise ValueError("this model was built for %d frequency bins (SpectConfig: sample_rate * window_size / 2 + 1), got input "
                              "with %d" % (F0, x.shape[2]))
-        y1 = ops.conv1_fwd(x, w1k, b1.detach(), lens_dev, Tp, dtype)
+        xb = ops.conv1_image(x) if dtype == torch.bfloat16 and F0 == 161 else None
+        if xb is not None:
+            y1 = ops.conv1_fwd_img(xb, N, T, w1k, b1.detach(), lens_dev, Tp)
+        else:
+            y1 = ops.conv1_fwd(x, w1k, b1.detach(), lens_dev, Tp, dtype)
         R1 = N * F1 * Tp
         a1 = torch.empty_like(y1)
         sv1 = ops.bn_fwd(y1, 1, training, g1.detach(), be1.detach(), bn1.running_mean, bn1.running_var,
@@ -276,12 +280,12 @@
                          bn2.num_batches_tracked, R2, 32, 32, x0, rld, F=F2, Tp=Tp, N=N, lens=lens_dev, eps=bn2.eps,
                          momentum=bn2.momentum)
         ctx.mod, ctx.dims, ctx.sv = mod, (N, T, Tp, dtype), (sv1, sv2)
-        ctx.save_for_backward(x, y1, a1, y2, lens_dev, w2)
+        ctx.save_for_backward(x, y1, a1, y2, lens_dev, w2, xb)
         return x0
 
     @staticmethod
     def backward(ctx, dx0):
-        x, y1, a1, y2, lens_dev, w2 = ctx.saved_tensors
+        x, y1, a1, y2, lens_dev, w2, xb = ctx.saved_tensors
         N, T, Tp, dtype = ctx.dims
         sv1, sv2 = ctx.sv
         c = ctx.mod._cache
@@ -289,16 +293,14 @@
         F0, F1, F2, rld = ctx.mod._F0, ctx.mod._F1, ctx.mod._F2, ctx.mod._rnn_ld
         R1, R2 = N * F1 * Tp, N * F2 * Tp
         dy2 = torch.empty_like(y2)
-        dg2, dbe2 = ops.bn_bwd(dx0, y2, dy2, 2, sv2, R2, 32, rld, 32, 32, F=F2, Tp=Tp, N=N, lens=lens_dev)
+        dg2, dbe2, db2 = ops.bn_bwd(dx0, y2, dy2, 2, sv2, R2, 32, rld, 32, 32, F=F2, Tp=Tp, N=N, lens=lens_dev, want_bias_grad=True)
         w2d = c.get(("w2d", dtype), [w2], lambda: [
             w2.detach()[:, :, q::2, :].flip(2, 3).permute(2, 3, 1, 0).contiguous().to(dtype) for q in (0, 1)])
         da1 = ops.conv2_dgrad(dy2, w2d[0], w2d[1], F0)
         dy1 = torch.empty_like(y1)
-        dg1, dbe1 = ops.bn_bwd(da1, y1, dy1, 1, sv1, R1, 32, 32, 32, 32, F=F1, Tp=Tp, N=N, lens=lens_dev)
-        db1 = ops.colsum(dy1.view(R1, 32))
-        dw1k = ops.conv1_wgrad(x, dy1, Tp)
+        dg1, dbe1, db1 = ops.bn_bwd(da1, y1, dy1, 1, sv1, R1, 32, 32, 32, 32, F=F1, Tp=Tp, N=N, lens=lens_dev, want_bias_grad=True)
+        dw1k = ops.conv1_wgrad_img(xb, N, T, dy1, Tp) if xb is not None else ops.conv1_wgrad(x, dy1, Tp)
         dw1 = dw1k.t().reshape(32, 1, 41, 11).contiguous()
-        db2 = ops.colsum(dy2.view(R2, 32))
         dw2 = ops.conv2_wgrad(dy2, a1, F0).view(21, 11, 32, 32).permute(2, 3, 0, 1).contiguous()
         return (None, dw1, db1, dg1, dbe1, dw2, db2, dg2, dbe2, None, None, None, None, None)
 
diff --git a/deepspeech/pytorch_amd/ops.py b/deepspeech/pytorch_amd/ops.py
--- a/deepspeech/pytorch_amd/ops.py
+++ b/deepspeech/pytorch_amd/ops.py
@@ -376,10 +376,15 @@
     return sv
 
 
-def bn_bwd(G, X, DX, mode, sv, R, Cc, ldg, ldx, lddx, F=0, Tp=0, N=0, lens=None):
+def bn_bwd(G, X, DX, mode, sv, R, Cc, ldg, ldx, lddx, F=0, Tp=0, N=0, lens=None, want_bias_grad=False):
     dgamma = torch.empty(Cc, dtype=torch.float32, device=X.device)
     dbeta = torch.empty(Cc, dtype=torch.float32, device=X.device)
     ws = torch.empty((2 * query("ds2_norm_partials", R) + 2) * Cc, dtype=torch.float32, device=X.device)
+    if want_bias_grad:
+        dbias = torch.empty(Cc, dtype=torch.float32, device=X.device)
+        call("ds2_bn_bwd_bias", dt(X), mode, P(G), P(X), P(DX), R, Cc, ldg, ldx, lddx, F, Tp, N, P(lens), P(sv.mean), P(sv.rstd),
+             P(sv.scale), P(sv.shift), P(dgamma), P(dbeta), P(dbias), P(ws), S())
+        return dgamma, dbeta, dbias
     call("ds2_bn_bwd", dt(X), mode, P(G), P(X), P(DX), R, Cc, ldg, ldx, lddx, F, Tp, N, P(lens), P(sv.mean), P(sv.rstd),
          P(sv.scale), P(sv.shift), P(dgamma), P(dbeta), P(ws), S())
     return dgamma, dbeta
@@ -402,6 +407,32 @@
     dw = torch.empty((451, 32), dtype=torch.float32, device=x.device)
     ws = torch.empty(query("ds2_conv1_wgrad_ws_floats", N, F0, Tp), dtype=torch.float32, device=x.device)
     call("ds2_conv1_wgrad", dt(dy1), P(x), P(dy1), P(dw), N, F0, T, Tp, P(ws), S())
+    return dw
+
+
+def conv1_image(x, out=None):
+    N, _, F0, T = x.shape
+    nbytes = query("ds2_conv1_image_bytes", N, F0, T)
+    if nbytes <= 0:
+        raise ValueError("the conv1 input image exists for 161 frequency bins only, got %d" % F0)
+    if out is None:
+        out = torch.empty(nbytes, dtype=torch.uint8, device=x.device)
+    assert out.dtype == torch.uint8 and out.numel() == nbytes and out.is_contiguous()
+    call("ds2_conv1_image", PF(x), P(out), N, F0, T, S())
+    return out
+
+
+def conv1_fwd_img(xb, N, T, w1k, b1, lens, Tp):
+    y1 = torch.empty((N, 81, Tp, 32), dtype=torch.bfloat16, device=xb.device)
+    call("ds2_conv1_fwd_img", P(xb), PF(w1k), PF(b1), P(lens), P(y1), N, T, Tp, S())
+    return y1
+
+
+def conv1_wgrad_img(xb, N, T, dy1, Tp):
+    assert dy1.dtype == torch.bfloat16
+    dw = torch.empty((451, 32), dtype=torch.float32, device=xb.device)
+    ws = torch.empty(query("ds2_conv1_wgrad_ws_floats", N, 161, Tp), dtype=torch.float32, device=xb.device)
+    call("ds2_conv1_wgrad_img", P(xb), P(dy1), P(dw), N, T, Tp, P(ws), S())
     return dw
 
 
diff --git a/include/ds2hip.h b/include/ds2hip.h
--- a/include/ds2hip.h
+++ b/include/ds2hip.h
@@ -61,6 +61,10 @@
                int F, int Tp, int N, const int* lens, const float* save_mean, const float* save_rstd,
                const float* save_scale, const float* save_shift, float* dgamma, float* dbeta, float* ws,
                ds2_stream_t stream);
+int ds2_bn_bwd_bias(int dtype, int mode, const void* G, const void* X, void* DX, long R, int C, long ldg, long ldx, long lddx,
+                    int F, int Tp, int N, const int* lens, const float* save_mean, const float* save_rstd,
+                    const float* save_scale, const float* save_shift, float* dgamma, float* dbeta, float* dbias, float* ws,
+                    ds2_stream_t stream);
 int ds2_colsum(int dtype, const void* X, long R, int C, long ld, float* out, float scale, float* ws, ds2_stream_t stream);
 
 int ds2_conv_rows(int F0, int* F1, int* F2);
@@ -69,6 +73,11 @@
 long ds2_conv1_wgrad_ws_floats(int N, int F0, int Tp);
 int ds2_conv1_wgrad(int dtype, const float* x, const void* dy1, float* dw1k, int N, int F0, int T, int Tp, float* ws,
                     ds2_stream_t stream);
+long ds2_conv1_image_bytes(int N, int F0, int T);
+int ds2_conv1_image(const float* x, void* xb, int N, int F0, int T, ds2_stream_t stream);
+int ds2_conv1_fwd_img(const void* xb, const float* w1k, const float* b1, const int* lens, void* y1, int N, int T, int Tp,
+                      ds2_stream_t stream);
+int ds2_conv1_wgrad_img(const void* xb, const void* dy1, float* dw1k, int N, int T, int Tp, float* ws, ds2_stream_t stream);
 long ds2_conv2_fwd_ws_bytes(int dtype, int N, int F0, int Tp);
 int ds2_conv2_fwd(int dtype, const void* a1, const void* w2t, const float* b2, const int* lens, void* y2, int N, int F0, int Tp,
                   void* ws, ds2_stream_t stream);
```

After: 21910, median of 6. Within noise of the previous version (+0.8%).
